# IRIS-AUDIO/SELD

Measured on AMD Instinct MI355X. Metric: train-step clips/sec (7ch×3000×64) seldnet.json at 1/2/4/8 MI355X, higher is better.
Workload: dtype f32; 1 GPU; model_config/seldnet.json train step (fwd+BCE/MSE+bwd+Adam), 32 clips/GPU of [T=3000,F=64,C=7], n_classes=12; global_batch=32, parallelism=dp1, dp_backend=none

## Files before the change

### seld_amd/csrc/api.hip

```cpp
#include "ctx.h"

#include <algorithm>
#include <math.h>
#include <stdio.h>
#include <string.h>

static std::string g_create_err;

int fail(seld_ctx* c, int code, const std::string& msg) {
    if (c) c->err = msg; else g_create_err = msg;
    return code;
}

static void add_var(std::vector<Var>& v, int64_t& off, const std::string& name, std::initializer_list<int64_t> shape) {
    Var x;
    x.name = name;
    x.off = off;
    x.rank = (int)shape.size();
    int64_t n = 1;
    int i = 0;
    for (int k = 0; k < 4; ++k) x.shape[k] = 1;
    for (auto s : shape) { x.shape[i++] = s; n *= s; }
    off += n;
    v.push_back(x);
// ... 357 lines not shown
        return fail(nullptr, SELD_ERR_HIP, "side stream / event creation failed");
    }
    for (int i = 0; i < a->n_gru; ++i)
        if (hipEventCreateWithFlags(&c->ev_bucket[i], hipEventDisableTiming) != hipSuccess) {
            seld_destroy(c);
            return fail(nullptr, SELD_ERR_HIP, "event creation failed");
        }
    ALLOC(c->sync_buf, (resn ? 16 * 128 : 128) + 1);
    for (int hd = 0; hd < 2; ++hd)
        for (auto& D : c->heads[hd].layers) {
            ALLOC(D.y, rows * (size_t)D.out); ALLOC(D.dy, rows * (size_t)D.out);
            if (D.ks > 1) ALLOC(D.xe, rows * (size_t)D.in);
            if (D.rate > 0.f) ALLOC(D.yd, rows * (size_t)D.out);
        }
    {
        size_t tmp = 0;
        for (int hd = 0; hd < 2; ++hd) for (auto& D : c->heads[hd].layers) if (D.ks > 1) tmp = std::max(tmp, rows * (size_t)D.in);
        if (tmp) ALLOC(c->head_tmp, tmp);
        if (a->output_coupling) ALLOC(c->doa_v1, rows * (size_t)(3 * a->n_classes));
    }
    {
        size_t ne = 0;
        for (int i = 0; i < a->n_gru; ++i) ne += 4 * gemm_sb_split_elems(c->gru[i].in_feat, 384);
        for (int hd = 0; hd < 2; ++hd) ne += 2 * gemm_sb_split_elems(c->heads[hd].layers[0].in, c->heads[hd].layers[0].out);
        ALLOC(c->gsplit, ne);
        unsigned short* q = c->gsplit;
        for (int i = 0; i < a->n_gru; ++i)
            for (int d = 0; d < 2; ++d) {
                c->ksp_fwd[i][d] = q; q += gemm_sb_split_elems(c->gru[i].in_feat, 384);
                c->ksp_bwd[i][d] = q; q += gemm_sb_split_elems(c->gru[i].in_feat, 384);
            }
        for (int hd = 0; hd < 2; ++hd) {
            const DenseL& D = c->heads[hd].layers[0];
            c->h0sp_fwd[hd] = q; q += gemm_sb_split_elems(D.in, D.out);
            c->h0sp_bwd[hd] = q; q += gemm_sb_split_elems(D.in, D.out);
        }
    }
    {
        const int nt = c->heads[0].layers.back().out + c->heads[1].layers.back().out, k = c->heads[0].layers[0].in;
        ALLOC(c->weff, (size_t)(k + 1) * nt);
        ALLOC(c->dy_all, rows * (size_t)nt);
        ALLOC(c->headF, (size_t)k * nt + nt);
    }
    ALLOC(c->loss_scratch, (size_t)loss_scratch_floats((int)rows));
    ALLOC(c->den_dev, 4); ALLOC(c->loss_out, rows + 4);
#undef ALLOC
    { int rc_ = v2_tables_create(c); if (rc_) { g_create_err = c->err; seld_destroy(c); return rc_; } }
    if (hipDeviceSynchronize() != hipSuccess) { seld_destroy(c); return fail(nullptr, SELD_ERR_HIP, "device sync after allocation failed"); }
    *out = c;
    return SELD_OK;
}

void seld_destroy(seld_ctx* c) {
    if (!c) return;
    hipSetDevice(c->device);
    hipDeviceSynchronize();
    for (auto& t : c->timers) for (auto e : t.ev) hipEventDestroy(e);
    for (auto e : c->ev_pool) hipEventDestroy(e);
    if (c->ev_fork) hipEventDestroy(c->ev_fork);
    if (c->ev_join) hipEventDestroy(c->ev_join);
    if (c->ev_prep) hipEventDestroy(c->ev_prep);
    if (c->ev_gram) hipEventDestroy(c->ev_gram);
    if (c->ev_rn_ready) hipEventDestroy(c->ev_rn_ready);
    for (auto e_ : c->ev_rn_free) if (e_) hipEventDestroy(e_);
    for (auto e : c->ev_bucket) if (e) hipEventDestroy(e);
    seld_dp_destroy(c);
    if (c->side) hipStreamDestroy(c->side);
    for (void* p : c->allocs) hipFree(p);
    delete c;
}

int seld_set_stream(seld_ctx* c, void* s) { if (!c) return SELD_ERR_INVALID; c->stream = (hipStream_t)s; return SELD_OK; }
int seld_set_batch(seld_ctx* c, int B) {
    if (!c) return SELD_ERR_INVALID;
    if (B < 1 || B > c->Bmax) return fail(c, SELD_ERR_INVALID, "batch exceeds the size given to seld_create");
    c->B = B;
    return SELD_OK;
}
int seld_set_option(seld_ctx* c, const char* key, int value) {
    if (!c || !key) return SELD_ERR_INVALID;
    if (!strcmp(key, "conv64_split_bf16")) { c->conv64_split_bf16 = value != 0; return SELD_OK; }
    if (!strcmp(key, "gemm_split_bf16")) { c->gemm_split_bf16 = value != 0; return SELD_OK; }
    if (!strcmp(key, "heads_fused")) { c->heads_fused = value != 0; return SELD_OK; }
    if (!strcmp(key, "dropout_seed")) { c->dropout_seed = 0x5e1d5e1d00000000ull ^ (uint64_t)(unsigned)value; return SELD_OK; }
    if (!strcmp(key, "dropout_step")) { c->dropout_step = (unsigned)value; return SELD_OK; }
    if (!strcmp(key, "conv1_split_bf16")) { c->conv1_split_bf16 = value != 0; return SELD_OK; }
    if (!strcmp(key, "gram_bg_blocks") && value >= 16 && value <= 512) { c->gram_bg_blocks = value; return SELD_OK; }
    if (!strcmp(key, "conv1_pool_fused")) { c->conv1_pool_fused = value != 0; return SELD_OK; }
    if (!strcmp(key, "conv1_gram")) { c->conv1_gram = value != 0; return SELD_OK; }
    if (!strcmp(key, "gru_wgrad_batch")) { c->gru_wgrad_batch = value != 0; return SELD_OK; }
    if (!strcmp(key, "gru_din_first")) { c->gru_din_first = value != 0; return SELD_OK; }
    if (!strcmp(key, "conv2_pre_fused")) { c->conv2_pre_fused = value != 0; return SELD_OK; }
    if (!strcmp(key, "conv3_pre_fused")) { c->conv3_pre_fused = value != 0; return SELD_OK; }
    if (!strcmp(key, "gram_parts") && (value == 1 || value == 2)) { c->gram_parts = value; return SELD_OK; }
    if (!strcmp(key, "xc_fused_fwd")) { c->xc_fused_fwd = value != 0; return SELD_OK; }
    if (!strcmp(key, "rn_split_bf16")) { c->rn_split_bf16 = value != 0; return SELD_OK; }
    if (!strcmp(key, "rn_wgrad_side")) { c->rn_wgrad_side = value != 0; return SELD_OK; }
    if (!strcmp(key, "rn_implicit3x3")) { c->rn_implicit3x3 = value != 0; return SELD_OK; }
    if (!strcmp(key, "rn_epi_stats")) { c->rn_epi_stats = value != 0; return SELD_OK; }
    if (!strcmp(key, "rn_epi_add")) { c->rn_epi_add = value != 0; return SELD_OK; }
    if (!strcmp(key, "xc_wgrad_side")) { c->xc_wgrad_side = value != 0; return SELD_OK; }
    if (!strcmp(key, "xc_fused_pw_bwd")) { c->xc_fused_pw_bwd = value != 0; return SELD_OK; }
    if (!strcmp(key, "bwd_four_products")) { c->bwd_four_products = value != 0; return SELD_OK; }
    if (!strcmp(key, "tn_tile_blocks") && value >= 64 && value <= 4096) { c->tn_tile_blocks = value; return SELD_OK; }
    if (!strcmp(key, "gru_var")) {
        if (value < 0 || value > 255) return fail(c, SELD_ERR_INVALID, "gru_var: 0..255");
        c->gru_var = value; return SELD_OK;
    }
    if (!strcmp(key, "tn_lds_floor") && value >= 0 && value <= 100) { c->tn_lds_floor = value; return SELD_OK; }
    if (!strcmp(key, "conv64_dbuf")) { c->conv64_dbuf = value != 0; return SELD_OK; }
    if (!strcmp(key, "conv_wgrad_side")) { c->conv_wgrad_side = value != 0; return SELD_OK; }
    if (!strcmp(key, "dgrad_r8")) { c->dgrad_r8 = value != 0; return SELD_OK; }
    if (!strcmp(key, "prep_side")) { c->prep_side = value != 0; return SELD_OK; }
    if (!strcmp(key, "xc_nowait")) { c->xc_nowait = value != 0; return SELD_OK; }
    if (!strcmp(key, "xc_fused_bn_sums")) { c->xc_fused_bn_sums = value != 0; return SELD_OK; }
    if (!strcmp(key, "xc_fused_dw_bwd")) { c->xc_fused_dw_bwd = value != 0; return SELD_OK; }
    if (!strcmp(key, "xc_w16")) { c->xc_w16 = value != 0; return SELD_OK; }
    if (!strcmp(key, "xc_xcd_map")) { c->xc_xcd_map = value != 0; return SELD_OK; }
    if (!strcmp(key, "bf16_single")) { c->bf16_single = value != 0; return SELD_OK; }
    return fail(c, SELD_ERR_INVALID, std::string("unknown option: ") + key);
}
int seld_sync(seld_ctx* c) {
    if (!c) return SELD_ERR_INVALID;
    HIPCHK(c, hipStreamSynchronize(c->stream));
    return SELD_OK;
}

int64_t seld_param_count(const seld_ctx* c) { return c ? c->nparam : -1; }
int64_t seld_state_count(const seld_ctx* c) { return c ? c->nstate : -1; }
int seld_variable_count(const seld_ctx* c, int trainable) { return c ? (int)(trainable ? c->tr.size() : c->nt.size()) : -1; }
int seld_variable_info(const seld_ctx* c, int trainable, int index, char* name, int name_cap, int64_t* offset,
                       int32_t* rank, int64_t shape[4]) {
    if (!c) return SELD_ERR_INVALID;
    const std::vector<Var>& v = trainable ? c->tr : c->nt;
    if (index < 0 || index >= (int)v.size()) return SELD_ERR_INVALID;
    if (name && name_cap > 0) { strncpy(name, v[index].name.c_str(), name_cap - 1); name[name_cap - 1] = 0; }
    if (offset) *offset = v[index].off;
    if (rank) *rank = v[index].rank;
    if (shape) for (int k = 0; k < 4; ++k) shape[k] = v[index].shape[k];
    return SELD_OK;
}

static int copy_h2d(seld_ctx* c, float* dst, const float* src, int64_t n, int64_t expect) {
    if (!c || !src || n != expect) return fail(c, SELD_ERR_INVALID, "size mismatch in host->device copy");
    HIPCHK(c, hipStreamSynchronize(c->stream));
    HIPCHK(c, hipMemcpy(dst, src, (size_t)n * 4, hipMemcpyHostToDevice));
    return SELD_OK;
}
static int copy_d2h(seld_ctx* c, float* dst, const float* src, int64_t n, int64_t expect) {
    if (!c || !dst || n != expect) return fail(c, SELD_ERR_INVALID, "size mismatch in device->host copy");
    HIPCHK(c, hipStreamSynchronize(c->stream));
    HIPCHK(c, hipMemcpy(dst, src, (size_t)n * 4, hipMemcpyDeviceToHost));
    return SELD_OK;
}
int seld_set_weights_host(seld_ctx* c, const float* w, int64_t n) { return c ? copy_h2d(c, c->params, w, n, c->nparam) : SELD_ERR_INVALID; }
int seld_get_weights_host(seld_ctx* c, float* w, int64_t n) { return c ? copy_d2h(c, w, c->params, n, c->nparam) : SELD_ERR_INVALID; }
int seld_set_state_host(seld_ctx* c, const float* s, int64_t n) { return c ? copy_h2d(c, c->state, s, n, c->nstate) : SELD_ERR_INVALID; }
int seld_get_state_host(seld_ctx* c, float* s, int64_t n) { return c ? copy_d2h(c, s, c->state, n, c->nstate) : SELD_ERR_INVALID; }
int seld_get_grads_host(seld_ctx* c, float* g, int64_t n) { return c ? copy_d2h(c, g, c->grads, n, c->nparam) : SELD_ERR_INVALID; }
int seld_get_adam_host(seld_ctx* c, float* m, float* v, int64_t n) {
    if (!c) return SELD_ERR_INVALID;
    int rc = copy_d2h(c, m, c->adam_m, n, c->nparam);
    if (rc) return rc;
    return copy_d2h(c, v, c->adam_v, n, c->nparam);
}
int seld_set_adam_host(seld_ctx* c, const float* m, const float* v, int64_t n, int64_t step) {
    if (!c || step < 0) return SELD_ERR_INVALID;
    int rc = copy_h2d(c, c->adam_m, m, n, c->nparam);
    if (rc) return rc;
    rc = copy_h2d(c, c->adam_v, v, n, c->nparam);
    if (rc) return rc;
    c->adam_step = step;
    return SELD_OK;
}
void* seld_param_ptr(seld_ctx* c) { return c ? c->params : nullptr; }
void* seld_grad_ptr(seld_ctx* c) { return c ? c->grads : nullptr; }

int seld_forward(seld_ctx* c, const float* x, float* sed, float* doa, int training) {
    if (!c || !x) return SELD_ERR_INVALID;
    HIPCHK(c, hipSetDevice(c->device));
    return forward_impl(c, x, sed, doa, training, false);
}

static int run_losses(seld_ctx* c, const float* y_sed, const float* y_doa, const seld_loss_cfg* cfg, float* sloss,
                      float* dloss, bool want_grads, bool defer_finalize = false) {
    hipStream_t st = c->stream;
    const int rows = c->B * c->S, nc = c->arch.n_classes;
    if (cfg->doa_loss < SELD_DOA_MSE || cfg->doa_loss > SELD_DOA_MSLE) return fail(c, SELD_ERR_INVALID, "bad doa_loss");
    if (cfg->doa_loss == SELD_DOA_MMSE) {
        if (cfg->mmse_den > 0.f) {
            if (hipMemcpyAsync(c->den_dev, &cfg->mmse_den, 4, hipMemcpyHostToDevice, st) != hipSuccess)
                return fail(c, SELD_ERR_HIP, "den copy failed");
            hipStreamSynchronize(st);
        } else {
            launch_mmse_den(st, y_doa, c->den_dev, c->loss_scratch, rows, nc);
            if (want_grads && c->dp_comm && c->dp_world > 1 && dp_allreduce(c, c->den_dev, 1, SELD_DTYPE_F32, st)) return fail(c, SELD_ERR_HIP, "RCCL all-reduce of the MMSE denominator failed");
        }
    }
    float* sl = sloss ? sloss : c->loss_out;
    float* dl = dloss ? dloss : c->loss_out + 4;
    const bool lin = heads_lin(c);
    const int n0 = c->heads[0].layers.back().out, nt = n0 + c->heads[1].layers.back().out;
    launch_losses(st, c->heads[0].layers.back().y, c->arch.output_coupling ? c->doa_v1 : c->heads[1].layers.back().y, y_sed, y_doa, cfg->doa_loss, cfg->w_sed,
                  cfg->w_doa, cfg->sed_grad_scale, c->den_dev, sl, dl,
                  want_grads ? (lin ? c->dy_all : c->heads[0].layers.back().dy) : nullptr,
                  want_grads ? (lin ? c->dy_all + n0 : c->heads[1].layers.back().dy) : nullptr, c->loss_scratch, c->B, c->S, nc,
                  lin ? nt : 0, lin ? nt : 0, defer_finalize ? 1 : 0);
    if (want_grads && c->arch.output_coupling)
        launch_v1_couple_bwd(st, c->heads[0].layers.back().y, c->heads[1].layers.back().y, lin ? c->dy_all : c->heads[0].layers.back().dy,
                             lin ? nt : n0, lin ? c->dy_all + n0 : c->heads[1].layers.back().dy, lin ? nt : nt - n0, rows, nc);
    if (defer_finalize) { c->fin_sl = sl; c->fin_dl = dl; c->fin_doa_loss = cfg->doa_loss; }
    return check_launch(c, "losses");
}

int seld_mmse_den(seld_ctx* c, const float* y_doa, float* den) {
    if (!c || !y_doa || !den) return SELD_ERR_INVALID;
    HIPCHK(c, hipSetDevice(c->device));
    launch_mmse_den(c->stream, y_doa, den, c->loss_scratch, c->B * c->S, c->arch.n_classes);
    return check_launch(c, "mmse_den");
}

int seld_test_step(seld_ctx* c, const float* x, const float* y_sed, const float* y_doa, const seld_loss_cfg* cfg,
                   float* sed, float* doa, float* sloss, float* dloss) {
    if (!c || !x || !y_sed || !y_doa || !cfg) return SELD_ERR_INVALID;
    HIPCHK(c, hipSetDevice(c->device));
    int rc = forward_impl(c, x, sed, doa, 0, false);
    if (rc) return rc;
    return run_losses(c, y_sed, y_doa, cfg, sloss, dloss, false);
}

int seld_train_fwd_bwd(seld_ctx* c, const float* x, const float* y_sed, const float* y_doa, const seld_loss_cfg* cfg,
                       float* sed, float* doa, float* sloss, float* dloss) {
    if (!c || !x || !y_sed || !y_doa || !cfg) return SELD_ERR_INVALID;
    HIPCHK(c, hipSetDevice(c->device));
    int rc = forward_impl(c, x, sed, doa, 1, true);
    if (rc) return rc;
    rc = run_losses(c, y_sed, y_doa, cfg, sloss, dloss, true, true);
    if (rc) return rc;
    return backward_impl(c, x);
}

int seld_adam_step(seld_ctx* c, float lr, float beta1, float beta2, float eps, int agc) {
    if (!c) return SELD_ERR_INVALID;
    HIPCHK(c, hipSetDevice(c->device));
    if (agc)
        for (auto& v : c->tr) launch_agc(c->stream, c->params, c->grads, v.off, v.rank, v.shape, nullptr);
    c->adam_step += 1;
    const double t = (double)c->adam_step;
    const float lr_t = (float)((double)lr * sqrt(1.0 - pow((double)beta2, t)) / (1.0 - pow((double)beta1, t)));
    PROF2(c, "adam");
    launch_adam(c->stream, c->params, c->grads, c->adam_m, c->adam_v, c->nparam, lr_t, beta1, beta2, eps);
    return check_launch(c, "adam");
}

int seld_train_step(seld_ctx* c, const float* x, const float* y_sed, const float* y_doa, const seld_loss_cfg* cfg,
                    float lr, int agc, float* sed, float* doa, float* sloss, float* dloss) {
    int rc = seld_train_fwd_bwd(c, x, y_sed, y_doa, cfg, sed, doa, sloss, dloss);
    if (rc) return rc;
    return seld_adam_step(c, lr, 0.9f, 0.999f, 1e-7f, agc);
}

int seld_debug_pool_routing(seld_ctx* c, int block, unsigned char* pos, unsigned char* gate) {
    if (c && pos && gate && c->arch.first_kind == SELD_FIRST_XCEPTION && block == (int)c->conv.size()) {
        HIPCHK(c, hipSetDevice(c->device));
        if (launch_pool_routing(c->stream, c->xc_x.back(), c->xc_feat, nullptr, c->xc_ident + 128, c->xc_ident + 192, pos, gate, c->B, c->S, 16, 1, 8))
            return fail(c, SELD_ERR_UNSUPPORTED, "pool_routing");
        HIPCHK(c, hipStreamSynchronize(c->stream));
        return check_launch(c, "pool_routing");
    }
    if (!c || !pos || !gate || block < 0 || block >= (int)c->conv.size()) return SELD_ERR_INVALID;
    HIPCHK(c, hipSetDevice(c->device));
    const ConvL& L = c->conv[block];
    const bool recorded = block == 0 && L.amax && (c->gram_active || (L.pf == 4 && (L.pt == 5 || L.pt == 4 || L.pt == 2 || L.pt == 1)));
    if (launch_pool_routing(c->stream, L.z, L.p, recorded ? L.amax : nullptr, L.scale, L.shift, pos, gate, c->B, L.H, L.W, L.pt, L.pf))
        return fail(c, SELD_ERR_UNSUPPORTED, "pool_routing");
    HIPCHK(c, hipStreamSynchronize(c->stream));
    return check_launch(c, "pool_routing");
}

static int set_override(seld_ctx* c, int kind, int block, int which, int64_t n, const int64_t* idx_host, const unsigned char* val_host, int64_t limit) {
    HIPCHK(c, hipSetDevice(c->device));
    HIPCHK(c, hipStreamSynchronize(c->stream));
    for (size_t i = 0; i < c->overrides.size();)
        if (c->overrides[i].kind == kind && c->overrides[i].block == block && c->overrides[i].which == which) c->overrides.erase(c->overrides.begin() + i);
        else ++i;
    if (n <= 0) return SELD_OK;
    if (!idx_host || !val_host) return SELD_ERR_INVALID;
    for (int64_t k = 0; k < n; ++k)
        if (idx_host[k] < 0 || idx_host[k] >= limit) return fail(c, SELD_ERR_INVALID, "injected decision index out of range");
    seld_ctx::Override o{kind, block, which, n, nullptr, nullptr};
    if (dalloc(c, &o.idx, (size_t)n) || dalloc(c, &o.val, (size_t)n)) return SELD_ERR_NOMEM;
    HIPCHK(c, hipMemcpy(o.idx, idx_host, (size_t)n * sizeof(int64_t), hipMemcpyHostToDevice));
    HIPCHK(c, hipMemcpy(o.val, val_host, (size_t)n, hipMemcpyHostToDevice));
    c->overrides.push_back(o);
    return SELD_OK;
}

int seld_debug_set_routing(seld_ctx* c, int block, int64_t n, const int64_t* idx_host, const unsigned char* val_host) {
    if (c && c->arch.first_kind == SELD_FIRST_XCEPTION && block == (int)c->conv.size()) {
        for (int64_t k = 0; k < n && val_host; ++k)
            if (val_host[k] > 8) return fail(c, SELD_ERR_INVALID, "injected routing value exceeds 1 + the window size");
        return set_override(c, 3, block, 0, n, idx_host, val_host, (int64_t)c->Bmax * c->S * 2 * 64);
    }
    if (!c || block < 0 || block >= (int)c->conv.size()) return SELD_ERR_INVALID;
    const ConvL& L = c->conv[block];
    const int64_t limit = (int64_t)c->Bmax * (L.H / L.pt) * (L.W / L.pf) * 64;
    for (int64_t k = 0; k < n && val_host; ++k)
        if (val_host[k] > L.pt * L.pf) return fail(c, SELD_ERR_INVALID, "injected routing value exceeds 1 + the window size");
    return set_override(c, 0, block, 0, n, idx_host, val_host, limit);
}

int seld_debug_set_relu_gates(seld_ctx* c, int block, int which, int64_t n, const int64_t* idx_host, const unsigned char* val_host) {
    if (!c || which < 0 || which > 2) return SELD_ERR_INVALID;
    if (c->arch.first_kind == SELD_FIRST_XCEPTION) {
        if (block < 0 || block >= (int)c->xc.size() || which != 0) return SELD_ERR_INVALID;
        return set_override(c, 2, block, 0, n, idx_host, val_host, (int64_t)c->Bmax * c->S * 16 * 64);
    }
    if (c->arch.first_kind != SELD_FIRST_RESNET50 || block < 0 || block >= (int)c->rn.size()) return SELD_ERR_INVALID;
    const RnBlock& R = c->rn[block];
    const int64_t limit = (int64_t)c->Bmax * c->S * R.Wout * (which == 2 ? 4 * R.w : R.w);
// ... 68 lines not shown
```

### seld_amd/csrc/backward.hip

```cpp
#include "ctx.h"

#include <algorithm>
#include <stdio.h>

static void wgrad_dense(seld_ctx* c, hipStream_t st, float* slab, const float* A, int lda, const float* Bm, int ldb, int M,
                        int K1, int N, int64_t w_off, int64_t b_off, int S, int shift) {
    int ns = 0;
    const int64_t cap = tn_slab_capacity() / ((int64_t)K1 * N + N);
    if (c->gemm_split_bf16 && gemm_tn_sb_usable(A, lda, Bm, ldb, K1, N)) launch_gemm_tn_sb(st, A, lda, Bm, ldb, slab, &ns, M, N, S, shift, 1);
    else launch_gemm_tn(st, A, lda, Bm, ldb, slab, &ns, M, K1, N, S, shift, 1, (int)std::min<int64_t>(cap, gemm_tn_max_splits()));
    launch_reduce_slabs2(st, slab, ns, (int64_t)K1 * N + N, c->grads + w_off, (int64_t)K1 * N, c->grads + b_off, N);
}

static void rn_bn_bwd(seld_ctx* c, hipStream_t st, RnConv& cv, const float* dy, const unsigned char* gate4, float* dz, int64_t M) {
    int nbx = 0;
    const int gate_z = gate4 ? 2 : 1;
    const float* mask = reinterpret_cast<const float*>(gate4);
    launch_rn_bn_bwd_reduce(st, cv.z, dy, mask, cv.coef, c->rn_part, &nbx, M, cv.Cout, gate_z);
    if (c->sync_fn) {
        const int nd = (cv.Cout + 63) / 64 * 128;
        launch_rn_bn_bwd_finalize(st, c->rn_part, nbx, (double)M, c->grads + cv.g_off, c->grads + cv.be_off, cv.coef, cv.Cout, c->sync_buf, 1);
        if (c->sync_fn(c->sync_user, c->sync_buf, nd + 1, SELD_DTYPE_F64, st)) { c->sync_failed = true; return; }
        launch_rn_bn_bwd_finalize(st, c->rn_part, nbx, 0.0, c->grads + cv.g_off, c->grads + cv.be_off, cv.coef, cv.Cout, c->sync_buf, 2);
    } else
        launch_rn_bn_bwd_finalize(st, c->rn_part, nbx, (double)M, c->grads + cv.g_off, c->grads + cv.be_off, cv.coef, cv.Cout);
    launch_rn_bn_bwd_dz(st, cv.z, dy, mask, cv.coef, dz, M, cv.Cout, gate_z);
}

static void heads_lin_side(seld_ctx* c, int rows) {
    const DenseL& S0 = c->heads[0].layers[0];
    const GruL& Glast = c->gru.back();
    const int nt = c->heads[0].layers[1].out + c->heads[1].layers[1].out, K = S0.in;
    int ns = 0;
    launch_gemm_tn(c->side, Glast.out, K, c->dy_all, nt, c->tn_slab_side, &ns, rows, K, nt, 0, 0, 1);
    launch_reduce_slabs2(c->side, c->tn_slab_side, ns, (int64_t)K * nt + nt, c->headF, (int64_t)K * nt, c->headF + (size_t)K * nt, nt);
    const float *w1[2], *b1[2], *w2[2];
    float *dw1[2], *db1[2], *dw2[2], *db2[2];
    int n[2];
    for (int hd = 0; hd < 2; ++hd) {
        const DenseL &L0 = c->heads[hd].layers[0], &L1 = c->heads[hd].layers[1];
        w1[hd] = c->params + L0.w_off; b1[hd] = c->params + L0.b_off; w2[hd] = c->params + L1.w_off;
        dw1[hd] = c->grads + L0.w_off; db1[hd] = c->grads + L0.b_off; dw2[hd] = c->grads + L1.w_off; db2[hd] = c->grads + L1.b_off;
        n[hd] = L1.out;
    }
    launch_heads_grad(c->side, w1, b1, w2, dw1, db1, dw2, db2, n, K, S0.out, c->headF, c->headF + (size_t)K * nt);
}

static int apply_overrides(seld_ctx* c) {
    hipStream_t st = c->stream;
    for (const auto& o : c->overrides) {
        if (o.kind == 0) {
            ConvL& L = c->conv[o.block];
            const bool recorded = o.block == 0 && L.amax && (c->gram_active || (L.pf == 4 && (L.pt == 5 || L.pt == 4 || L.pt == 2 || L.pt == 1)));
            if (!recorded && !L.z) return fail(c, SELD_ERR_UNSUPPORTED, "seld_debug_set_routing: this block keeps neither recorded positions nor its pre-BN tensor");
            launch_pool_routing_patch(st, L.z, L.p, recorded ? L.amax : nullptr, L.scale, L.shift, o.idx, o.val, o.n, L.H, L.W, L.pt, L.pf);
        } else if (o.kind == 2) {
            const int b = o.block / 3, u = o.block % 3;
            const bool fold = c->xc_fused_fwd && u > 0;
            if (fold) launch_relu_gate_patch_z(st, c->xc[o.block - 1].z, nullptr, c->xc[o.block - 1].scale, c->xc[o.block - 1].scale + 64, 64, o.idx, o.val, o.n);
            else launch_relu_gate_patch(st, u == 0 ? c->xc_x[b] : c->xc[o.block - 1].a, nullptr, o.idx, o.val, o.n);
        } else if (o.kind == 3) {
            launch_pool_routing_patch(st, c->xc_x.back(), c->xc_feat, nullptr, c->xc_ident + 128, c->xc_ident + 192, o.idx, o.val, o.n, c->S, 16, 1, 8);
        } else {
            RnBlock& R = c->rn[o.block];
            if (o.which == 2) launch_relu_gate_patch(st, R.out, R.gate, o.idx, o.val, o.n);
            else {
                RnConv& K = R.c[o.which];
                launch_relu_gate_patch_z(st, K.z, o.which == 0 ? R.y0 : R.y1, K.coef + 2 * K.Cout, K.coef + 3 * K.Cout, K.Cout, o.idx, o.val, o.n);
            }
        }
    }
    return SELD_OK;
}

static int backward_heads(seld_ctx* c) {
    hipStream_t st = c->stream;
    const int rows = c->B * c->S;
    GruL& Glast = c->gru.back();
    PROF2(c, "heads_bwd");
    float* dfeat = c->feat_grad;
    DenseL &S0 = c->heads[0].layers[0], &D0 = c->heads[1].layers[0];
    if (heads_lin(c)) {
        const int nt = c->heads[0].layers[1].out + c->heads[1].layers[1].out, K = S0.in;
        launch_gemm(st, c->dy_all, nt, c->weff, nt, nullptr, dfeat, K, rows, K, nt, 1, 0, 0);
    } else if (heads_general(c)) {
        for (int hd = 0; hd < 2; ++hd) {
            Head& Hd = c->heads[hd];
            for (int j = (int)Hd.layers.size() - 1; j >= 0; --j) {
                DenseL& D = Hd.layers[j];
                float* din = j == 0 ? dfeat : Hd.layers[j - 1].dy;
                const int accumulate = (j == 0 && hd == 1) ? 1 : 0;
                if (D.ks > 1) {
                    launch_gemm(st, D.dy, D.out, c->params + D.w_off, D.out, nullptr, c->head_tmp, D.in, rows, D.in, D.out, 1, 0, 0);
                    launch_time_fold(st, c->head_tmp, din, c->B, c->S, D.in_base, D.ks, accumulate);
                } else {
                    launch_gemm(st, D.dy, D.out, c->params + D.w_off, D.out, nullptr, din, D.in, rows, D.in, D.out, 1, 0, accumulate);
                }
                if (j > 0) {
                    const DenseL& P = Hd.layers[j - 1];
                    const int64_t n = (int64_t)rows * P.out;
                    if (P.rate > 0.f && c->last_training) launch_dropout(st, din, din, n, P.rate, c->dropout_seed, P.drop_id, c->dropout_cur);
                    if (Hd.hidden_act) launch_act_bwd(st, P.y, din, n, Hd.hidden_act);
                }
            }
        }
        fork_side(c);
        for (int hd = 0; hd < 2; ++hd) {
            Head& Hd = c->heads[hd];
            for (int j = (int)Hd.layers.size() - 1; j >= 0; --j) {
                DenseL& D = Hd.layers[j];
                const float* ain = D.ks > 1 ? D.xe
                                 : (j == 0 ? Glast.out : (Hd.layers[j - 1].rate > 0.f && c->last_training ? Hd.layers[j - 1].yd : Hd.layers[j - 1].y));
                wgrad_dense(c, c->side, c->tn_slab_side, ain, D.in, D.dy, D.out, rows, D.in, D.out, D.w_off, D.b_off, 0, 0);
            }
        }
    } else {
    const bool merged0 = S0.in == D0.in && S0.out == D0.out && (S0.out & 31) == 0;
    for (int hd = 0; hd < 2; ++hd) {
        Head& Hd = c->heads[hd];
        for (int j = (int)Hd.layers.size() - 1; j >= (merged0 ? 1 : 0); --j) {
            DenseL& D = Hd.layers[j];
            float* din = j == 0 ? dfeat : Hd.layers[j - 1].dy;
            const int accumulate = (j == 0 && hd == 1) ? 1 : 0;
            launch_gemm(st, D.dy, D.out, c->params + D.w_off, D.out, nullptr, din, D.in, rows, D.in, D.out, 1, 0, accumulate);
            if (j > 0 && Hd.hidden_act) launch_act_bwd(st, Hd.layers[j - 1].y, din, (int64_t)rows * D.in, Hd.hidden_act);
        }
    }
    if (merged0 && heads_sb(c) && gemm_sb_usable(S0.dy, S0.out, S0.in, S0.out) && gemm_sb_usable(D0.dy, S0.out, S0.in, S0.out)) {
        BwdFourScope four_;
        launch_gemm_sb(st, S0.dy, D0.dy, S0.out, c->h0sp_bwd[0], c->h0sp_bwd[1], nullptr, nullptr, dfeat, nullptr, S0.in, rows, S0.in,
                       S0.out, 0, 2);
    } else if (merged0)
        launch_gemm_dual_k(st, S0.dy, D0.dy, S0.out, c->params + S0.w_off, c->params + D0.w_off, S0.out, nullptr, dfeat, S0.in, rows,
                           S0.in, S0.out, 1, 0, 0);
    fork_side(c);
    for (int hd = 0; hd < 2; ++hd) {
        Head& Hd = c->heads[hd];
        for (int j = (int)Hd.layers.size() - 1; j >= 0; --j) {
            DenseL& D = Hd.layers[j];
            const float* ain = j == 0 ? Glast.out : Hd.layers[j - 1].y;
            wgrad_dense(c, c->side, c->tn_slab_side, ain, D.in, D.dy, D.out, rows, D.in, D.out, D.w_off, D.b_off, 0, 0);
        }
    }
    }
    return SELD_OK;
}

static int backward_gru(seld_ctx* c, const float* dfeat, const float** din) {
    hipStream_t st = c->stream;
    const int B = c->B, S = c->S, rows = B * S;
    const float* dout = dfeat;
    for (int i = (int)c->gru.size() - 1; i >= 0; --i) {
        GruL& G = c->gru[i];
        const bool conv_drop = c->last_training && c->arch.conv_dropout > 0.f, gru_drop = c->last_training && c->arch.gru_dropout > 0.f;
        const float* lin = i == 0 ? (c->arch.first_kind == SELD_FIRST_XCEPTION ? c->xc_feat : (c->arch.first_kind == SELD_FIRST_RESNET50 ? c->rn.back().out : (conv_drop ? c->conv.back().pd : c->conv.back().p))) : c->gru[i - 1].out;
        {
            PROF(c, "gru_bwd");
            if (gru_drop) {
// ... 369 lines not shown
```

### seld_amd/csrc/common.h

```cpp
#pragma once
#include <hip/hip_runtime.h>
#include <stdint.h>
#include "../../include/seld_hip.h"

inline int ok() { return hipGetLastError() == hipSuccess ? SELD_OK : SELD_ERR_HIP; }

typedef float f32x16 __attribute__((ext_vector_type(16)));

#define MFMA_F32_32x32x2(a, b, c) __builtin_amdgcn_mfma_f32_32x32x2f32((a), (b), (c), 0, 0, 0)

__device__ __forceinline__ int mfma_row(int r, int hi) { return (r & 3) + 8 * (r >> 2) + 4 * hi; }

__device__ __forceinline__ f32x16 zero16() {
    f32x16 z;
#pragma unroll
    for (int i = 0; i < 16; ++i) z[i] = 0.f;
    return z;
}
__device__ __forceinline__ float dpp_quad_xor1(float v) {
    return __int_as_float(__builtin_amdgcn_update_dpp(0, __float_as_int(v), 0xB1 , 0xF, 0xF, true));
}
__device__ __forceinline__ float dpp_quad_xor2(float v) {
    return __int_as_float(__builtin_amdgcn_update_dpp(0, __float_as_int(v), 0x4E , 0xF, 0xF, true));
}
// ... 152 lines not shown
int launch_rn_product_fwd(hipStream_t st, const float* A, int lda, const float* w, const unsigned short* wsp, float* z, int M, int K, int N,
                          float* stat_part = nullptr, int* nbx = nullptr, size_t part_cap = 0);
int launch_rn_product_dgrad(hipStream_t st, const float* dz, const float* w, const unsigned short* wsp_t, float* dA, int ldd, int M, int K, int N,
                            int accumulate, const float* addg = nullptr, const unsigned char* gate4 = nullptr);
int launch_rn_product_wgrad(hipStream_t st, const float* A, int lda, const float* dz, float* slab, int64_t slab_cap, float* dw, int M, int K, int N,
                            int split_bf16);
int launch_rn_w32_embed(hipStream_t st, const float* w, float* w2);
int launch_rn_w32_extract(hipStream_t st, const float* dw2, float* dw);
int rn_conv3_sb_ok(int C, int N);
int launch_rn_conv3_fwd(hipStream_t st, const float* img, const unsigned short* wsp, float* z, int B, int H, int W, int C, int N,
                        float* stat_part = nullptr, int* nbx = nullptr, size_t part_cap = 0);
int launch_rn_conv3_dgrad(hipStream_t st, const float* dz, const unsigned short* wsp_flip, float* dimg, int B, int H, int W, int C, int N);
int launch_rn_conv3_wgrad(hipStream_t st, const float* img, const float* dz, float* slab, int64_t slab_cap, float* dw, int B, int H, int W, int C, int N);
int launch_xc_unit_fwd(hipStream_t st, const float* x, const float* kdw, const float* wpw, float* dwo, float* z, float* partial, int* npartial,
                       int B, int H, int W, const float* aff = nullptr);
int xc_partial_capacity();
int launch_dw3x3_fwd(hipStream_t st, const float* x, const float* k, float* y, int B, int H, int W, const float* aff = nullptr);
int launch_dw3x3_bwd_data(hipStream_t st, const float* dy, const float* k, const float* xin, const float* add, float* dx, int B, int H, int W,
                          const float* aff = nullptr);
int launch_dw3x3_bwd_w(hipStream_t st, const float* x, const float* dy, float* slab, int* nslab, int B, int H, int W, const float* aff = nullptr);
int xc_dw_fused_slabs(int B, int H);
int launch_dw3x3_bwd_fused(hipStream_t st, const float* dy, const float* k, const float* xin, const float* add, float* dx, float* slab, int* nslab,
                           int B, int H, int W, const float* aff = nullptr, const float* bn_mean = nullptr, const float* bn_invstd = nullptr,
                           float* bn_partial = nullptr);
int launch_xc_fold_partials(hipStream_t st, const float* partial, int n, float* out, int* nout);
int launch_xc_bn_stats(hipStream_t st, const float* z, float* partial, int* npartial, int64_t npix);
int launch_xc_bn_bwd_reduce(hipStream_t st, const float* z, const float* dy, const float* mean, const float* invstd, float* partial,
                            int* npartial, int64_t npix);
int launch_xc_bn_apply(hipStream_t st, const float* z, const float* scale, const float* shift, const float* res, float* out, int64_t npix);
int xc_pw_bwd_slabs();
int launch_xc_pw_bwd(hipStream_t st, const float* z, const float* gy, const float* dwo, const float* wpw, const float* mean, const float* invstd,
                     const float* scale, const float* c1c2, float* f1, float* slab, int* nslab, int64_t npix);
int launch_xc_bn_bwd_dz(hipStream_t st, const float* z, const float* dy, const float* mean, const float* invstd, const float* scale,
                        const float* c1c2, float* dz, int64_t npix);
int launch_xc_ident(hipStream_t st, float* ident);
int launch_bn_partials_to_sums(hipStream_t st, const float* partial, int npartial, double* sums, double local_count);
int launch_bn_finalize_sums(hipStream_t st, const double* sums, double count, const float* gamma, const float* beta,
                            float* mov_mean, float* mov_var, float* mean, float* invstd, float* scale, float* shift);
int launch_bn_bwd_local(hipStream_t st, const double* sums, float* dgamma, float* dbeta);
int launch_bn_bwd_c1c2(hipStream_t st, const double* sums, double count, float* c1c2);
int launch_pool_routing_patch(hipStream_t st, float* z, float* p, unsigned char* amax, const float* scale, const float* shift,
                              const int64_t* idx, const unsigned char* val, int64_t n, int H, int W, int pt, int pf);
int launch_relu_gate_patch_z(hipStream_t st, float* z, float* y, const float* scale, const float* shift, int C, const int64_t* idx,
                             const unsigned char* val, int64_t n);
int launch_affine_copy(hipStream_t st, const float* x, const float* aff, float* dst, int64_t n, int C);
int launch_relu_gate_patch(hipStream_t st, float* y, unsigned char* gate_bits, const int64_t* idx, const unsigned char* val, int64_t n);
int launch_pool_routing(hipStream_t st, const float* z, const float* p, const unsigned char* amax, const float* scale,
                        const float* shift, unsigned char* pos, unsigned char* gate, int B, int H, int W, int pt, int pf);
int launch_bn_pool_bwd_dz(hipStream_t st, const float* z, const float* dp, const float* mean, const float* invstd,
                          const float* scale, const float* shift, const float* c1c2, float* dz,
                          int B, int H, int W, int C, int pt, int pf);
int bn_partial_capacity();

struct GemmEpi { float* stat_part = nullptr; const float* addg = nullptr; const unsigned char* gate4 = nullptr; };
extern thread_local GemmEpi g_gemm_epi;
struct GemmEpiScope {
    GemmEpiScope(float* stat_part, const float* addg = nullptr, const unsigned char* gate4 = nullptr) { g_gemm_epi.stat_part = stat_part; g_gemm_epi.addg = addg; g_gemm_epi.gate4 = gate4; }
    ~GemmEpiScope() { g_gemm_epi = GemmEpi(); }
};
int gemm_epi_row_blocks(int M, int split_bf16);
int launch_gemm(hipStream_t st, const float* A, int lda, const float* Bm, int ldb, const float* bias, float* C,
                int ldc, int M, int N, int K, int transb, int act, int accumulate);
int launch_gemm_dual_n(hipStream_t st, const float* A, int lda, const float* B0, const float* B1, int ldb, const float* bias0,
                       const float* bias1, float* C0, float* C1, int ldc, int M, int N, int K, int transb, int act);
int launch_gemm_mirror(hipStream_t st, const float* A, int lda, const float* Bm, int ldb, const float* bias, float* C, float* mirror,
                       int ldc, int M, int N, int K, int transb, int act);
int launch_gemm_heads(hipStream_t st, const float* A, int lda, const float* Bm, const float* bias, float* C0, float* C1, float* M0,
                      float* M1, int M, int n0, int n1, int K, int act0, int act1);
int launch_heads_weff(hipStream_t st, const float* const* w1, const float* const* b1, const float* const* w2, const float* const* b2,
                      const int* n, int K, int Hd, float* weff);
int launch_heads_grad(hipStream_t st, const float* const* w1, const float* const* b1, const float* const* w2, float* const* dw1,
                      float* const* db1, float* const* dw2, float* const* db2, const int* n, int K, int Hd, const float* F,
                      const float* cs);
int launch_gemm_dual_k(hipStream_t st, const float* A0, const float* A1, int lda, const float* B0, const float* B1, int ldb,
                       const float* bias, float* C, int ldc, int M, int N, int K, int transb, int act, int accumulate);
extern int g_gsb_dbg;
size_t gemm_sb_split_elems(int K, int N);
int gemm_sb_usable(const void* A, int lda, int N, int K);
int launch_gemm_split_b(hipStream_t st, int njobs, const float* const* src, unsigned short* const* dst, const int* ldb,
                        const int* transb, const int* K, const int* N);
int launch_gemm_sb(hipStream_t st, const float* A0, const float* A1, int lda, const unsigned short* Bs0, const unsigned short* Bs1,
                   const float* bias0, const float* bias1, float* C0, float* C1, int ldc, int M, int N, int K, int act, int mode,
                   int accum = 0,
                   int conv_C = 0, int conv_H = 0, int conv_W = 0);
int launch_gemm_tn(hipStream_t st, const float* A, int lda, const float* Bm, int ldb, float* slab, int* nslab,
                   int M, int K1, int N, int S, int shift, int want_bias, int max_splits = 0, int chunk_rows = 32);
int gemm_tn_sb_usable(const void* A, int lda, const void* Bm, int ldb, int K1, int N);
#define TN_MAX_JOBS 4
struct TnJobs {
    const float* A[TN_MAX_JOBS];
    const float* B[TN_MAX_JOBS];
    int lda[TN_MAX_JOBS], shift[TN_MAX_JOBS];
    float* out_w[TN_MAX_JOBS];
    float* out_b[TN_MAX_JOBS];
};
int launch_gemm_tn_sb_batch(hipStream_t st, const TnJobs& jobs, int njobs, int ldb, float* slab, int* nslab, int M, int N, int S, int want_bias);
int launch_reduce_slabs2_batch(hipStream_t st, const float* slab, int nslab, int64_t stride, const TnJobs& jobs, int njobs, int64_t n_w, int64_t n_b);
int launch_gemm_tn_sb(hipStream_t st, const float* A, int lda, const float* Bm, int ldb, float* slab, int* nslab, int M, int N, int S,
                      int shift, int want_bias);
int launch_gemm_tn_sb_tiles(hipStream_t st, const float* A, int lda, const float* Bm, int ldb, float* slab, int64_t slab_cap, int* nslab,
                            int M, int K1, int N, int conv_C = 0, int conv_H = 0, int conv_W = 0);
int launch_reduce_slabs2(hipStream_t st, const float* slab, int nslab, int64_t stride, float* out_w, int64_t n_w,
                         float* out_b, int64_t n_b);
int gemm_tn_max_splits();
inline int64_t tn_slab_capacity() { return (int64_t)gemm_tn_max_splits() * (384 * 384 + 384); }
int launch_colsum(hipStream_t st, const float* X, int ld, float* slab, int* nslab, int M, int N);

int launch_gru_fwd(hipStream_t st, const float* gx_f, const float* gx_b, const float* U_f, const float* U_b,
                   const float* brec_f, const float* brec_b, float* h_f, float* h_b, float* sv_f, float* sv_b,
                   int B, int S, const float* rm_f = nullptr, const float* rm_b = nullptr, float* hm_f = nullptr, float* hm_b = nullptr);
int launch_gru_fwd_df(hipStream_t st, const float* gx_f, const float* gx_b, const float* U_f, const float* U_b,
                      const float* brec_f, const float* brec_b, float* h_f, float* h_b, float* sv_f, float* sv_b, int B, int S);
int gru_df_trace_read(int which, unsigned long long* out);
int launch_gru_bwd(hipStream_t st, const float* dout, const float* h_f, const float* h_b, const float* sv_f,
                   const float* sv_b, const float* U_f, const float* U_b, float* dgx_f, float* dgx_b,
                   float* dgh_f, float* dgh_b, int B, int S, const float* rm_f = nullptr, const float* rm_b = nullptr, const float* hm_f = nullptr,
                   const float* hm_b = nullptr);
int gru_timing_read(int which, unsigned long long* out, int blocks);
int launch_gru_fwd_uni(hipStream_t st, const float* gx, const float* U, const float* brec, float* h, float* sv, int B, int S);
int launch_gru_bwd_dh(hipStream_t st, const float* dh_f, const float* dh_b, const float* h_f, const float* h_b, const float* sv_f, const float* sv_b,
                      const float* U_f, const float* U_b, float* dgx_f, float* dgx_b, float* dgh_f, float* dgh_b, int B, int S);
int launch_lstm_fwd(hipStream_t st, const float* gx_f, const float* gx_b, const float* U_f, const float* U_b, float* h_f, float* h_b,
                    float* c_f, float* c_b, float* sv_f, float* sv_b, int B, int S);
int launch_lstm_bwd(hipStream_t st, const float* dh_f, const float* dh_b, const float* c_f, const float* c_b, const float* sv_f,
                    const float* sv_b, const float* U_f, const float* U_b, float* dgx_f, float* dgx_b, int B, int S);
int launch_mul(hipStream_t st, const float* a, const float* b, float* out, int64_t n);

struct seld_loss_cfg;
int launch_act_bwd(hipStream_t st, const float* y, float* dy, int64_t n, int act);
int launch_time_expand(hipStream_t st, const float* x, float* xe, int B, int S, int C, int ks);
int launch_time_fold(hipStream_t st, const float* dxe, float* dx, int B, int S, int C, int ks, int accumulate);
int launch_dropout(hipStream_t st, const float* in, float* out, int64_t n, float rate, uint64_t seed, unsigned layer, unsigned step);
int launch_mask_rows(hipStream_t st, const float* in, const float* mask, float* out, int64_t rows, int S, int F, int accumulate);
int launch_fill(hipStream_t st, float* out, int64_t n, float v);
int launch_v1_couple_fwd(hipStream_t st, const float* sed, const float* doa1, float* out, float* out2, int rows, int nc);
int launch_v1_couple_bwd(hipStream_t st, const float* sed, const float* doa1, float* dsed_pre, int ld_sed, float* ddoa_pre, int ld_doa, int rows, int nc);
int launch_mmse_den(hipStream_t st, const float* y_doa, float* den, float* scratch, int rows, int nc);
int launch_losses(hipStream_t st, const float* sed, const float* doa, const float* y_sed, const float* y_doa,
                  int doa_loss, float w_sed, float w_doa, float sed_grad_scale, const float* den_dev,
                  float* sloss, float* dloss, float* dsed_pre, float* ddoa_pre, float* scratch, int B, int S, int nc, int ld_sed = 0,
                  int ld_doa = 0, int defer_finalize = 0);
int launch_losses_finalize(hipStream_t st, int doa_loss, const float* den_dev, float* sloss, float* dloss, float* scratch, int B, int S,
                           int nc);
int loss_scratch_floats(int rows);
int launch_adam(hipStream_t st, float* theta, const float* g, float* m, float* v, int64_t n, float lr_t,
                float beta1, float beta2, float eps);
int launch_agc(hipStream_t st, const float* theta, float* g, int64_t off, int rank, const int64_t* shape,
               float* scratch);
```

### seld_amd/csrc/ctx.h

```cpp
#pragma once
#include "common.h"
#include "../../include/seld_hip.h"

#include <string>
#include <vector>

struct Var { std::string name; int64_t off; int rank; int64_t shape[4]; };

struct Timer { std::string name; std::vector<hipEvent_t> ev; int64_t launches = 0; double ms = 0.0; };

struct ConvL {
    int H, W, Cin, pt, pf;
    int64_t w_off, b_off, g_off, be_off;
    int64_t mm_off, mv_off;
    float *z = nullptr, *p = nullptr, *dp = nullptr;
    float* pd = nullptr;
    unsigned char* amax = nullptr;
    float* zext = nullptr;
    float *mean, *invstd, *scale, *shift, *c1c2;
};

struct GruL {
    int in_feat;
    int64_t k_off[2], u_off[2], b_off[2];
// ... 13 lines not shown
    unsigned short *wsp = nullptr, *wsp_t = nullptr;
    unsigned short *wsp9 = nullptr, *wsp9_flip = nullptr;
    float *w2 = nullptr, *dw2 = nullptr;
};
struct RnBlock {
    int Cin, w, stride_f, Win, Wout;
    bool proj;
    RnConv c[3], sc;
    float *y0 = nullptr, *y1 = nullptr, *out = nullptr;
    unsigned char* gate = nullptr;
};

struct XcUnit {
    int64_t dw_off, pw_off, g_off, be_off;
    int64_t mm_off, mv_off;
    float *dwo = nullptr, *z = nullptr, *a = nullptr;
    float *mean, *invstd, *scale, *shift, *c1c2;
};

struct Head {
    std::vector<DenseL> layers;
    int act;
    int hidden_act = 0;
};

struct seld_ctx {
    seld_arch arch;
    int B, Bmax, T, S, device;
    hipStream_t stream = nullptr;
    std::vector<Var> tr, nt;
    int64_t nparam = 0, nstate = 0;
    float *params = nullptr, *grads = nullptr, *adam_m = nullptr, *adam_v = nullptr, *state = nullptr;
    int64_t adam_step = 0;
    std::vector<ConvL> conv;
    std::vector<GruL> gru;
    struct Override { int kind, block, which; int64_t n; int64_t* idx; unsigned char* val; };
    std::vector<Override> overrides;
    Head heads[2];
    std::vector<XcUnit> xc;
    std::vector<float*> xc_x;
    float *xc_small = nullptr, *xc_ident = nullptr, *xc_feat = nullptr, *xc_part = nullptr, *xc_slab = nullptr;
    float* xc_unit_slab = nullptr;
    size_t xc_unit_slab_per = 0, xc_unit_slab_pw = 0, xc_unit_slab_dw = 0;
    int xc_nowait = 1;
    float* xc_slab_tmp = nullptr;
    float* xc_part_dw = nullptr;
    size_t xc_slab_per = 0;
    float *xc_g[4] = {}, *xc_dz2 = nullptr;
    int xc_fused_pw_bwd = 1;
    int xc_wgrad_side = 1;
    std::vector<RnBlock> rn;
    float *rn_part = nullptr, *rn_part_side = nullptr, *rn_gx[2] = {}, *rn_bz[2] = {}, *rn_ba = nullptr, *rn_bb[3] = {}, *rn_bcol = nullptr;
    size_t rn_part_floats = 0;
    hipEvent_t ev_rn_ready = nullptr, ev_rn_free[5] = {};
    float* rn_w9_slab = nullptr;
    int rn_wgrad_side = 1;
    size_t rn_col_elems = 0;
    int rn_implicit3x3 = 1;
    int rn_feat = 0;
    float *feat_grad = nullptr;
    float *dzbuf = nullptr, *small = nullptr, *stat_partial = nullptr, *bn_partial = nullptr;
    float *wgrad_slab = nullptr, *tn_slab = nullptr, *cs_slab = nullptr, *wflip = nullptr;
    float *wgrad_slab_side = nullptr, *dzbuf_alt = nullptr;
    int conv_wgrad_side = 1;
    int dgrad_r8 = 1;
    float *dgx[SELD_MAX_LAYERS][2] = {}, *dgh[SELD_MAX_LAYERS][2] = {};
    float* tn_slab_side = nullptr;
    unsigned short* wsplit = nullptr;
    unsigned short *wsp_fwd[SELD_MAX_LAYERS] = {}, *wsp_bwd[SELD_MAX_LAYERS] = {};
    int conv1_gram = 1;
    bool xc_fused_fwd = true;
    int gram_parts = 2;
    bool conv3_pre_fused = true;
    bool conv2_pre_fused = true;
    bool gru_din_first = false;
    bool gru_wgrad_batch = true;
    bool gram_active = false;
    float *gram_slab = nullptr, *gram = nullptr, *mmat = nullptr;
    hipEvent_t ev_gram = nullptr;
    int conv1_split_bf16 = 1;
    int conv1_pool_fused = 1;
    int heads_fused = 1;
    float *weff = nullptr, *dy_all = nullptr, *headF = nullptr;
    int rn_split_bf16 = 1;
    int gemm_split_bf16 = 1;
    unsigned short* gsplit = nullptr;
    unsigned short *ksp_fwd[SELD_MAX_LAYERS][2] = {}, *ksp_bwd[SELD_MAX_LAYERS][2] = {}, *h0sp_fwd[2] = {}, *h0sp_bwd[2] = {};
    int conv64_split_bf16 = 1;
    hipStream_t side = nullptr;
    hipEvent_t ev_fork = nullptr, ev_join = nullptr, ev_prep = nullptr;
    int prep_side = 0;
    hipEvent_t ev_bucket[SELD_MAX_LAYERS] = {};
    seld_allreduce_fn sync_fn = nullptr;
    void* sync_user = nullptr;
    int sync_world = 1;
    double* sync_buf = nullptr;
    bool sync_failed = false;
    int bf16_single = 0;
    int bwd_four_products = 1, gru_var = 11, conv64_dbuf = 1, tn_tile_blocks = 384, tn_lds_floor = 0, gram_bg_blocks = 192;
    int xc_fused_bn_sums = 1;
    int xc_fused_dw_bwd = 1;
    int xc_w16 = 1;
    int xc_xcd_map = 1;
    int rn_epi_stats = 1;
    int rn_epi_add = 1;
    void* dp_comm = nullptr;
    int dp_rank = 0, dp_world = 1;
    hipStream_t dp_stream = nullptr;
    hipEvent_t ev_dp_main = nullptr, ev_dp_done = nullptr;
    float *dsed_pre = nullptr, *ddoa_pre = nullptr, *sed_int = nullptr, *doa_int = nullptr;
    float *doa_v1 = nullptr;
    float *head_tmp = nullptr;
    float* ones = nullptr;
    uint64_t dropout_seed = 0x5e1d5e1d5e1d5e1dull; unsigned dropout_step = 0, dropout_cur = 0; int last_training = 0;
    float *loss_scratch = nullptr, *den_dev = nullptr, *loss_out = nullptr;
    float *fin_sl = nullptr, *fin_dl = nullptr;
    int fin_doa_loss = 0;
    struct V2Tab { void *tiles = nullptr, *segs = nullptr; int32_t* reg = nullptr; float* scale = nullptr; int ntiles = 0, nsegs = 0; } v2;
    float *swa_w = nullptr, *swa_s = nullptr;
    int swa_cnt = 0;
    std::vector<void*> allocs;
    std::string err;
    int prof = 0;
    std::vector<Timer> timers;
    std::vector<hipEvent_t> ev_pool;
};

int fail(seld_ctx* c, int code, const std::string& msg);
int check_launch(seld_ctx* c, const char* what);

#define HIPCHK(c, expr)                                                                         \
    do {                                                                                        \
        hipError_t e_ = (expr);                                                                 \
        if (e_ != hipSuccess)                                                                   \
            return fail(c, SELD_ERR_HIP, std::string(#expr) + ": " + hipGetErrorString(e_));    \
    } while (0)

template <typename T>
int dalloc(seld_ctx* c, T** p, size_t n) {
    void* q = nullptr;
    hipError_t e = hipMalloc(&q, n * sizeof(T) + 256);
    if (e != hipSuccess) return fail(c, SELD_ERR_NOMEM, std::string("hipMalloc: ") + hipGetErrorString(e));
    c->allocs.push_back(q);
    *p = reinterpret_cast<T*>(q);
    return 0;
}

struct ProfScope {
    seld_ctx* c; int idx;
    ProfScope(seld_ctx* c_, const char* name, int level = 1) : c(c_), idx(-1) {
        if (c->prof < level) return;
        for (size_t i = 0; i < c->timers.size(); ++i) if (c->timers[i].name == name) idx = (int)i;
        if (idx < 0) { Timer t; t.name = name; c->timers.push_back(t); idx = (int)c->timers.size() - 1; }
        hipEvent_t e = take(c); hipEventRecord(e, c->stream); c->timers[idx].ev.push_back(e);
    }
    ~ProfScope() {
        if (idx < 0) return;
        hipEvent_t e = take(c); hipEventRecord(e, c->stream); c->timers[idx].ev.push_back(e);
        c->timers[idx].launches++;
    }
    static hipEvent_t take(seld_ctx* c) {
        if (c->ev_pool.empty()) { hipEvent_t e; hipEventCreate(&e); return e; }
        hipEvent_t e = c->ev_pool.back(); c->ev_pool.pop_back(); return e;
    }
};
#define PROF_CAT2(a, b) a##b
#define PROF_CAT(a, b) PROF_CAT2(a, b)
#define PROF(c, name) ProfScope PROF_CAT(prof_scope_, __LINE__)(c, name, 1)
#define PROF2(c, name) ProfScope PROF_CAT(prof_scope_, __LINE__)(c, name, 2)
#define PROF3(c, name) ProfScope PROF_CAT(prof_scope_, __LINE__)(c, name, 3)

void fork_side(seld_ctx* c);
void apply_kernel_choices(const seld_ctx* c);
bool gru_sb(const seld_ctx* c, const GruL& G);
bool heads_general(const seld_ctx* c);
bool heads_sb(const seld_ctx* c);
bool heads_lin(const seld_ctx* c);
bool rn_c1_implicit(const seld_ctx* c, const RnBlock& R);
int rn_c1_width(const RnBlock& R);
bool rn_c1_direct(const RnBlock& R);

int forward_impl(seld_ctx* c, const float* x, float* sed, float* doa, int training, bool save);
int backward_impl(seld_ctx* c, const float* x);

int v2_tables_create(seld_ctx* c);

int dp_allreduce(seld_ctx* c, void* buf, int64_t count, int dtype, hipStream_t st);
```

### seld_amd/csrc/forward.hip

```cpp
#include "ctx.h"

#include <stdio.h>

static int prepare_heads_weff(seld_ctx* c, hipStream_t st) {
    const float *w1[2], *b1[2], *w2[2], *b2[2];
    int n[2];
    for (int hd = 0; hd < 2; ++hd) {
        const DenseL &L0 = c->heads[hd].layers[0], &L1 = c->heads[hd].layers[1];
        w1[hd] = c->params + L0.w_off; b1[hd] = c->params + L0.b_off; w2[hd] = c->params + L1.w_off; b2[hd] = c->params + L1.b_off;
        n[hd] = L1.out;
    }
    return launch_heads_weff(st, w1, b1, w2, b2, n, c->heads[0].layers[0].in, c->heads[0].layers[0].out, c->weff);
}

static int prepare_gemm_splits(seld_ctx* c, hipStream_t st, bool with_grad_orientation) {
    const float* src[16]; unsigned short* dst[16]; int ldb[16], tb[16], K[16], N[16];
    int n = 0;
    auto flush = [&]() { int rc = n ? launch_gemm_split_b(st, n, src, dst, ldb, tb, K, N) : 0; n = 0; return rc; };
    auto add = [&](const float* w, unsigned short* d, int ld, int transb, int k, int nn) {
        src[n] = w; dst[n] = d; ldb[n] = ld; tb[n] = transb; K[n] = k; N[n] = nn;
        return ++n == 16 ? flush() : 0;
    };
    for (size_t i = 0; i < c->gru.size(); ++i) {
        const GruL& G = c->gru[i];
// ... 3 lines not shown
            if (with_grad_orientation && add(c->params + G.k_off[d], c->ksp_bwd[i][d], 384, 1, 384, G.in_feat)) return -1;
        }
    }
    if (heads_sb(c) && !heads_lin(c))
        for (int hd = 0; hd < 2; ++hd) {
            const DenseL& D = c->heads[hd].layers[0];
            if (add(c->params + D.w_off, c->h0sp_fwd[hd], D.out, 0, D.in, D.out)) return -1;
            if (with_grad_orientation && add(c->params + D.w_off, c->h0sp_bwd[hd], D.out, 1, D.out, D.in)) return -1;
        }
    return flush();
}

static void rn_bn(seld_ctx* c, hipStream_t st, RnConv& cv, int64_t M, int training, int nbx_have = 0, float* part = nullptr) {
    int nbx = nbx_have;
    if (!part) part = c->rn_part;
    if (training && !nbx_have) launch_rn_bn_stats(st, cv.z, part, &nbx, M, cv.Cout);
    float *g = c->params + cv.g_off, *be = c->params + cv.be_off, *mm = c->state + cv.mm_off, *mv = c->state + cv.mv_off;
    if (training && c->sync_fn) {
        const int nd = (cv.Cout + 63) / 64 * 128;
        launch_rn_bn_finalize(st, part, nbx, (double)M, g, be, mm, mv, cv.coef, cv.Cout, 1, c->sync_buf, 1);
        if (c->sync_fn(c->sync_user, c->sync_buf, nd + 1, SELD_DTYPE_F64, st)) { c->sync_failed = true; return; }
        launch_rn_bn_finalize(st, part, nbx, 0.0, g, be, mm, mv, cv.coef, cv.Cout, 1, c->sync_buf, 2);
        return;
    }
    launch_rn_bn_finalize(st, part, nbx, (double)M, g, be, mm, mv, cv.coef, cv.Cout, training);
}

static int heads_couple(seld_ctx* c, float* doa, int rows) {
    if (c->arch.output_coupling)
        launch_v1_couple_fwd(c->stream, c->heads[0].layers.back().y, c->heads[1].layers.back().y, c->doa_v1, doa, rows, c->arch.n_classes);
    return check_launch(c, "forward");
}

static void rn_weight_prep(seld_ctx* c, hipStream_t st, bool save) {
    const float* src[16]; unsigned short* dst[16]; int ldb[16], tb[16], Ks[16], Ns[16];
    int n = 0;
    auto add = [&](const float* w, unsigned short* d, int ld, int transb, int k, int nn) {
        src[n] = w; dst[n] = d; ldb[n] = ld; tb[n] = transb; Ks[n] = k; Ns[n] = nn;
        if (++n == 16) { launch_gemm_split_b(st, n, src, dst, ldb, tb, Ks, Ns); n = 0; }
    };
    for (auto& R : c->rn)
        for (RnConv* cv : {&R.c[0], &R.c[1], &R.c[2], &R.sc}) {
            const int K = cv->k * cv->k * cv->Cin, N = cv->Cout;
            if (cv->wsp) add(c->params + cv->w_off, cv->wsp, N, 0, K, N);
            if (cv->wsp_t && save) {
                if (cv == &R.c[1] && rn_c1_implicit(c, R)) add(c->params + cv->w_off, cv->wsp_t, N, 2, 9 * N, cv->Cin);
                else add(c->params + cv->w_off, cv->wsp_t, N, 1, N, K);
            }
        }
    if (n) launch_gemm_split_b(st, n, src, dst, ldb, tb, Ks, Ns);
    const float* w9[8]; unsigned short* d9[8]; int f9[8];
    n = 0;
    for (auto& R : c->rn) {
        if (!rn_c1_direct(R)) continue;
        const float* wsrc = c->params + R.c[1].w_off;
        if (R.c[1].w2) { launch_rn_w32_embed(st, wsrc, R.c[1].w2); wsrc = R.c[1].w2; }
        w9[n] = wsrc; d9[n] = R.c[1].wsp9; f9[n++] = 0;
        if (save) { w9[n] = wsrc; d9[n] = R.c[1].wsp9_flip; f9[n++] = 1; }
        if (n >= 7) { launch_split_weights_batch(st, n, w9, d9, f9); n = 0; }
    }
    if (n) launch_split_weights_batch(st, n, w9, d9, f9);
}

template <typename Layer>
static int bn_coeffs(seld_ctx* c, hipStream_t st, int training, const float* part, int np, double count, Layer& L) {
    const float *g = c->params + L.g_off, *be = c->params + L.be_off;
    float *mm = c->state + L.mm_off, *mv = c->state + L.mv_off;
    if (training && c->sync_fn) {
        launch_bn_partials_to_sums(st, part, np, c->sync_buf, count);
        if (c->sync_fn(c->sync_user, c->sync_buf, 129, SELD_DTYPE_F64, st)) return fail(c, SELD_ERR_HIP, "sync_bn all-reduce callback failed");
        launch_bn_finalize_sums(st, c->sync_buf, 0.0 , g, be, mm, mv, L.mean, L.invstd, L.scale, L.shift);
    } else if (training)
        launch_bn_finalize(st, part, np, count, g, be, mm, mv, L.mean, L.invstd, L.scale, L.shift, 64, 1);
    else
        launch_bn_eval_coeffs(st, g, be, mm, mv, L.scale, L.shift, 64);
    return SELD_OK;
}

struct FwdPass {
    const float* x;
    int training;
    bool save;
    bool conv_drop, gru_drop;
};

static int forward_weight_prep(seld_ctx* c, bool save, bool* prep_on_side, bool* rn_prep_on_side) {
    hipStream_t st = c->stream;
    *prep_on_side = false;
    *rn_prep_on_side = !c->rn.empty() && c->rn_split_bf16 && c->prep_side && c->ev_prep;
    if (*rn_prep_on_side) { fork_side(c); rn_weight_prep(c, c->side, save); hipEventRecord(c->ev_prep, c->side); }
    GemmSplitJobs a; SplitWeightJobs b; HeadsLin h;
    a.one = b.one = g_mfma_one;
    int na = 0, nb = 0;
    bool fits = true;
    auto adda = [&](const float* w, unsigned short* d, int ld, int transb, int k, int nn) {
        if (na == GSB_MAX_JOBS) { fits = false; return; }
        a.src[na] = w; a.dst[na] = d; a.ldb[na] = ld; a.transb[na] = transb; a.K[na] = k; a.N[na] = nn; ++na;
    };
    for (size_t i = 0; i < c->gru.size(); ++i) {
        const GruL& G = c->gru[i];
        if (!gru_sb(c, G)) continue;
        for (int d = 0; d < 2; ++d) {
            adda(c->params + G.k_off[d], c->ksp_fwd[i][d], 384, 0, G.in_feat, 384);
            if (save) adda(c->params + G.k_off[d], c->ksp_bwd[i][d], 384, 1, 384, G.in_feat);
        }
    }
    if (heads_sb(c) && !heads_lin(c))
        for (int hd = 0; hd < 2; ++hd) {
            const DenseL& D = c->heads[hd].layers[0];
            adda(c->params + D.w_off, c->h0sp_fwd[hd], D.out, 0, D.in, D.out);
            if (save) adda(c->params + D.w_off, c->h0sp_bwd[hd], D.out, 1, D.out, D.in);
        }
    a.njobs = na;
    static_assert(2 * (SELD_MAX_LAYERS - 1) <= 8, "the conv64 weight planes of a step fit one SplitWeightJobs");
    if (c->conv64_split_bf16)
        for (size_t i = 1; i < c->conv.size(); ++i) {
            b.w[nb] = c->params + c->conv[i].w_off; b.dst[nb] = c->wsp_fwd[i]; b.flip[nb++] = 0;
            if (save) { b.w[nb] = c->params + c->conv[i].w_off; b.dst[nb] = c->wsp_bwd[i]; b.flip[nb++] = 1; }
        }
    const bool lin = heads_lin(c);
    if (lin)
        for (int hd = 0; hd < 2; ++hd) {
            const DenseL &L0 = c->heads[hd].layers[0], &L1 = c->heads[hd].layers[1];
            h.w1[hd] = c->params + L0.w_off; h.b1[hd] = c->params + L0.b_off; h.w2[hd] = c->params + L1.w_off;
            h.b2[hd] = c->params + L1.b_off; h.n[hd] = L1.out;
            h.K = L0.in; h.Hd = L0.out;
        }
    if (fits && (!lin || h.K + 1 <= 4 * 144)) {
        *prep_on_side = c->prep_side && c->ev_prep && c->xc.empty() && c->rn.empty() && c->conv.size() >= 2;
        if (*prep_on_side) fork_side(c);
        if (launch_weight_prep(*prep_on_side ? c->side : st, a, na, b, nb, h, lin ? c->weff : nullptr)) return fail(c, SELD_ERR_UNSUPPORTED, "weight_prep");
        if (*prep_on_side) hipEventRecord(c->ev_prep, c->side);
    } else {
        if (prepare_gemm_splits(c, st, save)) return fail(c, SELD_ERR_UNSUPPORTED, "gemm_split_b");
        if (lin && prepare_heads_weff(c, st)) return fail(c, SELD_ERR_UNSUPPORTED, "heads_weff");
        if (nb && launch_split_weights_batch(st, nb, b.w, b.dst, b.flip)) return fail(c, SELD_ERR_UNSUPPORTED, "split_weights");
    }
    return SELD_OK;
}

static int forward_conv_blocks(seld_ctx* c, const FwdPass& p, bool prep_on_side, const float** feat) {
    hipStream_t st = c->stream;
    const int B = c->B;
    const float* in = p.x;
    bool pre_pending = false;
    for (size_t i = 0; i < c->conv.size(); ++i) {
        ConvL& L = c->conv[i];
        bool ext_now = false;
        int npart = 0;
        float* stat = p.training ? c->stat_partial : nullptr;
        char tn[32];
        snprintf(tn, sizeof tn, "conv%d_fwd", (int)i + 1);
        const bool fused_pool = i == 0 && c->conv1_pool_fused && L.pt == 5 && L.pf == 4 && L.W == 64;
        const bool gram = fused_pool && p.save && c->conv1_gram;
        if (i == 0) c->gram_active = gram;
        const bool pre_next = fused_pool && (gram || !p.save) && c->conv2_pre_fused && !p.conv_drop && c->arch.first_kind == SELD_FIRST_SIMPLE_CONV &&
                              i + 1 < c->conv.size() && c->conv64_split_bf16 && !g_mfma_one && conv64_fwd_sb_takes_pre(c->conv[i + 1].W);
        if (fused_pool) {
            PROF(c, tn);
            if (launch_conv_first_fwd_pool(st, in, c->params + L.w_off, c->params + L.b_off, c->params + L.g_off,
                                           (p.save && !gram) ? L.z : nullptr, (gram || pre_next) ? L.zext : L.p, p.save ? L.amax : nullptr, stat,
                                           &npart, B, L.H, L.Cin, c->conv1_split_bf16))
                return fail(c, SELD_ERR_UNSUPPORTED, "conv_first_fwd_pool");
        } else if (i == 0) {
            PROF(c, tn);
            if (launch_conv_first_fwd(st, in, c->params + L.w_off, c->params + L.b_off, L.z, stat, &npart, B, L.H, L.Cin))
                return fail(c, SELD_ERR_UNSUPPORTED, "conv_first_fwd");
// ... 84 lines not shown
        if (rn_prep_on_side) hipStreamWaitEvent(st, c->ev_prep, 0);
        else rn_weight_prep(c, st, p.save);
    }
    const float* X = *feat;
    int rc_ = 0;
    for (auto& R : c->rn) {
        if (c->sync_failed) break;
        const int64_t M = (int64_t)B * S * R.Wout;
        const int w = R.w;
        const bool sc_side = R.proj && c->rn_wgrad_side && !c->sync_fn;
        if (sc_side) {
            hipEventRecord(c->ev_rn_ready, st); hipStreamWaitEvent(c->side, c->ev_rn_ready, 0);
            int nb_ = 0;
            if (launch_rn_product_fwd(c->side, X, R.Cin * R.stride_f, c->params + R.sc.w_off, sb ? R.sc.wsp : nullptr, R.sc.z, (int)M, R.Cin, 4 * w,
                                      epi_stats ? c->rn_part_side : nullptr, &nb_, c->rn_part_floats))
                return fail(c, SELD_ERR_INVALID, "resnet50_block: projection shortcut product refused");
            rn_bn(c, c->side, R.sc, M, p.training, nb_, c->rn_part_side);
            hipEventRecord(c->ev_rn_free[0], c->side);
        }
        int nb0 = 0;
        { PROF3(c, "rn_products_fwd"); rc_ = launch_rn_product_fwd(st, X, R.Cin * R.stride_f, c->params + R.c[0].w_off, sb ? R.c[0].wsp : nullptr, R.c[0].z, (int)M, R.Cin, w,
                                                                   epi_stats ? c->rn_part : nullptr, &nb0, c->rn_part_floats); }
        if (rc_) return fail(c, SELD_ERR_INVALID, "resnet50_block: reduce convolution's product refused");
        { PROF3(c, "rn_bn_fwd"); rn_bn(c, st, R.c[0], M, p.training, nb0); }
        { PROF3(c, "rn_bn_fwd"); launch_rn_bn_apply(st, R.c[0].z, R.c[0].coef, nullptr, R.y0, M, w, 1); }
        if (sb && rn_c1_direct(R)) {
            int npart = 0;
            if (R.c[1].w2) {
                { PROF3(c, "rn_products_fwd"); launch_conv64_fwd_sb(st, R.y0, R.c[1].wsp9, nullptr, R.c[1].z, nullptr, nullptr, B, S, rn_c1_width(R)); }
                { PROF3(c, "rn_bn_fwd"); rn_bn(c, st, R.c[1], M, p.training); }
            } else {
                if (p.training && (size_t)conv_sb_partial_capacity() * 128 > c->rn_part_floats)
                    return fail(c, SELD_ERR_INVALID, "resnet50_block: more BatchNorm partials than rn_part holds");
                { PROF3(c, "rn_products_fwd"); launch_conv64_fwd_sb(st, R.y0, R.c[1].wsp9, nullptr, R.c[1].z, p.training ? c->rn_part : nullptr, &npart, B, S, R.Wout); }
                { PROF3(c, "rn_bn_fwd"); rn_bn(c, st, R.c[1], M, p.training, npart); }
            }
        } else if (sb && rn_c1_implicit(c, R)) {
            int nb1 = 0;
            { PROF3(c, "rn_products_fwd"); rc_ = launch_rn_conv3_fwd(st, R.y0, R.c[1].wsp, R.c[1].z, B, S, R.Wout, w, w, epi_stats ? c->rn_part : nullptr, &nb1,
                                                                     c->rn_part_floats); }
            if (rc_) return fail(c, SELD_ERR_INVALID, "resnet50_block: 3x3 convolution's product refused");
            { PROF3(c, "rn_bn_fwd"); rn_bn(c, st, R.c[1], M, p.training, nb1); }
        } else {
            if (!R.c[1].col && dalloc(c, &R.c[1].col, (size_t)M * 9 * w)) return fail(c, SELD_ERR_NOMEM, "im2col tensor");
            launch_im2col3x3(st, R.y0, R.c[1].col, B, S, R.Wout, w);
            int nb1 = 0;
            { PROF3(c, "rn_products_fwd"); rc_ = launch_rn_product_fwd(st, R.c[1].col, 9 * w, c->params + R.c[1].w_off, sb ? R.c[1].wsp : nullptr, R.c[1].z, (int)M, 9 * w, w,
                                                                       epi_stats ? c->rn_part : nullptr, &nb1, c->rn_part_floats); }
            if (rc_) return fail(c, SELD_ERR_INVALID, "resnet50_block: 3x3 convolution's product refused");
            { PROF3(c, "rn_bn_fwd"); rn_bn(c, st, R.c[1], M, p.training, nb1); }
        }
        { PROF3(c, "rn_bn_fwd"); launch_rn_bn_apply(st, R.c[1].z, R.c[1].coef, nullptr, R.y1, M, w, 1); }
        int nb2 = 0;
        { PROF3(c, "rn_products_fwd"); rc_ = launch_rn_product_fwd(st, R.y1, w, c->params + R.c[2].w_off, sb ? R.c[2].wsp : nullptr, R.c[2].z, (int)M, w, 4 * w,
                                                                   epi_stats ? c->rn_part : nullptr, &nb2, c->rn_part_floats); }
        if (rc_) return fail(c, SELD_ERR_INVALID, "resnet50_block: expand convolution's product refused");
        { PROF3(c, "rn_bn_fwd"); rn_bn(c, st, R.c[2], M, p.training, nb2); }
        if (R.proj) {
            if (sc_side) hipStreamWaitEvent(st, c->ev_rn_free[0], 0);
            else {
                int nbs = 0;
                { PROF3(c, "rn_products_fwd"); rc_ = launch_rn_product_fwd(st, X, R.Cin * R.stride_f, c->params + R.sc.w_off, sb ? R.sc.wsp : nullptr, R.sc.z, (int)M, R.Cin, 4 * w,
                                                                           epi_stats ? c->rn_part : nullptr, &nbs, c->rn_part_floats); }
                if (rc_) return fail(c, SELD_ERR_INVALID, "resnet50_block: projection shortcut product refused");
                { PROF3(c, "rn_bn_fwd"); rn_bn(c, st, R.sc, M, p.training, nbs); }
            }
            { PROF3(c, "rn_bn_fwd"); launch_rn_bn_apply2(st, R.c[2].z, R.c[2].coef, R.sc.z, R.sc.coef, R.out, M, 4 * w, p.save ? R.gate : nullptr); }
        } else {
            { PROF3(c, "rn_bn_fwd"); launch_rn_bn_apply(st, R.c[2].z, R.c[2].coef, X, R.out, M, 4 * w, 1, p.save ? R.gate : nullptr); }
        }
        X = R.out;
    }
    if (c->sync_failed) { c->sync_failed = false; return fail(c, SELD_ERR_HIP, "sync_bn all-reduce callback failed"); }
    *feat = X;
    return SELD_OK;
}

static int forward_gru(seld_ctx* c, const FwdPass& p, const float** feat_io) {
    hipStream_t st = c->stream;
    const int B = c->B, S = c->S, rows = B * S;
    const float* feat = *feat_io;
    const int gparts = !c->gram_active ? 0 : (c->gram_parts == 2 && c->gru.size() >= 2 ? 2 : 1);
    int gram_ns = 0;
    for (size_t i = 0; i < c->gru.size(); ++i) {
        GruL& G = c->gru[i];
        if (p.gru_drop) {
            PROF(c, "gru_fwd");
            const float rate = c->arch.gru_dropout;
            for (int d = 0; d < 2; ++d) {
                launch_dropout(st, c->ones, G.imask[d], (int64_t)B * G.in_feat, rate, c->dropout_seed, 96u + 4u * (unsigned)i + d, c->dropout_cur);
                launch_dropout(st, c->ones, G.rmask[d], (int64_t)B * 128, rate, c->dropout_seed, 98u + 4u * (unsigned)i + d, c->dropout_cur);
                launch_mask_rows(st, feat, G.imask[d], G.xm[d], rows, S, G.in_feat, 0);
                if (gru_sb(c, G) && gemm_sb_usable(G.xm[d], G.in_feat, 384, G.in_feat))
                    launch_gemm_sb(st, G.xm[d], nullptr, G.in_feat, c->ksp_fwd[i][d], nullptr, c->params + G.b_off[d], nullptr, G.gx[d], nullptr, 384, rows, 384,
                                   G.in_feat, 0, 0);
                else
                    launch_gemm(st, G.xm[d], G.in_feat, c->params + G.k_off[d], 384, c->params + G.b_off[d], G.gx[d], 384, rows, 384, G.in_feat, 0, 0, 0);
            }
            if (launch_gru_fwd(st, G.gx[0], G.gx[1], c->params + G.u_off[0], c->params + G.u_off[1], c->params + G.b_off[0] + 384,
                               c->params + G.b_off[1] + 384, G.h[0], G.h[1], G.sv[0], G.sv[1], B, S, G.rmask[0], G.rmask[1], G.hm[0], G.hm[1]))
                return fail(c, SELD_ERR_UNSUPPORTED, "gru_fwd (dropout)");
        } else {
        {
            PROF2(c, "gru_inproj_gemm");
            if (gru_sb(c, G) && gemm_sb_usable(feat, G.in_feat, 384, G.in_feat))
                launch_gemm_sb(st, feat, nullptr, G.in_feat, c->ksp_fwd[i][0], c->ksp_fwd[i][1], c->params + G.b_off[0],
                               c->params + G.b_off[1], G.gx[0], G.gx[1], 384, rows, 384, G.in_feat, 0, 1);
            else
                launch_gemm_dual_n(st, feat, G.in_feat, c->params + G.k_off[0], c->params + G.k_off[1], 384, c->params + G.b_off[0],
                                   c->params + G.b_off[1], G.gx[0], G.gx[1], 384, rows, 384, G.in_feat, 0, 0);
        }
        if ((int)i < gparts) fork_side(c);
        {
            PROF(c, "gru_fwd");
            launch_gru_fwd(st, G.gx[0], G.gx[1], c->params + G.u_off[0], c->params + G.u_off[1], c->params + G.b_off[0] + 384,
                           c->params + G.b_off[1] + 384, G.h[0], G.h[1], p.save ? G.sv[0] : nullptr, p.save ? G.sv[1] : nullptr, B, S);
        }
        }
        if ((int)i < gparts && p.gru_drop) fork_side(c);
        if ((int)i < gparts) {
            int ns = 0;
            const int kp = conv_gram_dim(c->conv[0].Cin);
            if (i == 0) gram_ns = 0;
            if (launch_conv_first_gram(c->side, p.x, c->gram_slab + (size_t)gram_ns * kp * kp, &ns, B, c->conv[0].H, c->conv[0].Cin, 1, (int)i, gparts))
                return fail(c, SELD_ERR_UNSUPPORTED, "conv_first_gram");
            gram_ns += ns;
            if ((int)i == gparts - 1) {
                launch_reduce_slabs(c->side, c->gram_slab, gram_ns, (int64_t)kp * kp, c->gram, (int64_t)kp * kp, 0);
                hipEventRecord(c->ev_gram, c->side);
            }
        }
        launch_mul(st, G.h[0], G.h[1], G.out, (int64_t)rows * 128);
        feat = G.out;
    }
    *feat_io = feat;
    return SELD_OK;
}

static int forward_heads(seld_ctx* c, const FwdPass& p, const float* feat, float* sed, float* doa) {
    hipStream_t st = c->stream;
    const int rows = c->B * c->S;
    {
        PROF2(c, "heads_fwd");
        DenseL &S0 = c->heads[0].layers[0], &D0 = c->heads[1].layers[0];
        if (heads_lin(c)) {
            DenseL &S1 = c->heads[0].layers[1], &D1 = c->heads[1].layers[1];
            const int nt = S1.out + D1.out;
            if (launch_gemm_heads(st, feat, S0.in, c->weff, c->weff + (size_t)S0.in * nt, S1.y, D1.y, sed, doa, rows, S1.out, D1.out,
                                  S0.in, c->heads[0].act, c->heads[1].act))
                return fail(c, SELD_ERR_UNSUPPORTED, "gemm_heads");
            return heads_couple(c, doa, rows);
        }
        if (heads_general(c)) {
            for (int hd = 0; hd < 2; ++hd) {
                const float* a = feat;
                Head& Hd = c->heads[hd];
                float* outp = hd == 0 ? sed : doa;
                for (size_t j = 0; j < Hd.layers.size(); ++j) {
                    DenseL& D = Hd.layers[j];
                    const bool lastl = (j + 1 == Hd.layers.size());
                    if (D.ks > 1) { launch_time_expand(st, a, D.xe, c->B, c->S, D.in_base, D.ks); a = D.xe; }
                    launch_gemm_mirror(st, a, D.in, c->params + D.w_off, D.out, c->params + D.b_off, D.y, lastl ? outp : nullptr, D.out,
                                       rows, D.out, D.in, 0, lastl ? Hd.act : Hd.hidden_act);
                    a = D.y;
                    if (!lastl && D.rate > 0.f && p.training) {
                        launch_dropout(st, D.y, D.yd, (int64_t)rows * D.out, D.rate, c->dropout_seed, D.drop_id, c->dropout_cur);
                        a = D.yd;
                    }
                }
            }
            return heads_couple(c, doa, rows);
        }
        const bool merged0 = c->heads[0].layers.size() > 1 && c->heads[1].layers.size() > 1 && S0.in == D0.in && S0.out == D0.out &&
                             c->heads[0].hidden_act == c->heads[1].hidden_act;
        const int hact0 = c->heads[0].hidden_act;
        if (merged0 && heads_sb(c) && gemm_sb_usable(feat, S0.in, S0.out, S0.in))
            launch_gemm_sb(st, feat, nullptr, S0.in, c->h0sp_fwd[0], c->h0sp_fwd[1], c->params + S0.b_off, c->params + D0.b_off, S0.y,
                           D0.y, S0.out, rows, S0.out, S0.in, hact0, 1);
        else if (merged0)
            launch_gemm_dual_n(st, feat, S0.in, c->params + S0.w_off, c->params + D0.w_off, S0.out, c->params + S0.b_off,
                               c->params + D0.b_off, S0.y, D0.y, S0.out, rows, S0.out, S0.in, 0, hact0);
        for (int hd = 0; hd < 2; ++hd) {
            const float* a = feat;
            Head& Hd = c->heads[hd];
            float* outp = hd == 0 ? sed : doa;
            for (size_t j = 0; j < Hd.layers.size(); ++j) {
                DenseL& D = Hd.layers[j];
                const bool lastl = (j + 1 == Hd.layers.size());
                float* y = D.y;
                if (!(merged0 && j == 0))
                    launch_gemm_mirror(st, a, D.in, c->params + D.w_off, D.out, c->params + D.b_off, y, lastl ? outp : nullptr, D.out,
                                       rows, D.out, D.in, 0, lastl ? Hd.act : Hd.hidden_act);
                a = y;
            }
        }
    }
    return heads_couple(c, doa, rows);
}

int forward_impl(seld_ctx* c, const float* x, float* sed, float* doa, int training, bool save) {
    apply_kernel_choices(c);
    c->last_training = training;
    if (training) c->dropout_cur = c->dropout_step++;
    const FwdPass p = {x, training, save, training && c->arch.conv_dropout > 0.f, training && c->arch.gru_dropout > 0.f};
    if (p.gru_drop && !save) return fail(c, SELD_ERR_UNSUPPORTED, "gru_dropout: a training forward without saved gates");
    bool prep_on_side = false, rn_prep_on_side = false;
    const float* feat = nullptr;
    int rc = forward_weight_prep(c, save, &prep_on_side, &rn_prep_on_side);
    if (!rc) rc = forward_conv_blocks(c, p, prep_on_side, &feat);
    if (!rc && c->arch.first_kind == SELD_FIRST_XCEPTION) rc = forward_xception(c, p, &feat);
    if (!rc && c->arch.first_kind == SELD_FIRST_RESNET50) rc = forward_resnet(c, p, rn_prep_on_side, &feat);
    if (!rc) rc = forward_gru(c, p, &feat);
    if (!rc) rc = forward_heads(c, p, feat, sed, doa);
    return rc;
}
```

### seld_amd/csrc/gemm.hip

```cpp
#include "common.h"
#include "prep.h"

#define GT_LDA 65

template <int TRANSB>
__global__ __launch_bounds__(256) void gemm_f32_kernel(const float* __restrict__ A, int lda,
                                                       const float* __restrict__ Bm, int ldb,
                                                       const float* __restrict__ bias, float* __restrict__ C,
                                                       int ldc, int M, int N, int K, int act, int accumulate,
                                                       const float* __restrict__ A1, const float* __restrict__ B1,
                                                       const float* __restrict__ bias1, float* __restrict__ C1, int mode,
                                                       float* __restrict__ M0, float* __restrict__ M1, int nsplit, GemmEpi epi) {
    const int ntx = (N + 63) >> 6;
    const bool second = mode == 1 && (int)blockIdx.x >= ntx;
    if (second) { Bm = B1; bias = bias1; C = C1; }
    constexpr int LDB = TRANSB ? 65 : 64;
    __shared__ __attribute__((aligned(16))) float As[32 * GT_LDA];
    __shared__ __attribute__((aligned(16))) float Bs[32 * LDB];
    const int tid = threadIdx.x, lane = tid & 63, wave = tid >> 6;
    const int hi = lane >> 5, li = lane & 31;
    const int wr = wave >> 1, wc = wave & 1;
    const int m0 = blockIdx.y * 64, n0 = (second ? (int)blockIdx.x - ntx : (int)blockIdx.x) * 64;
    const bool a_vec = ((lda & 3) == 0) && ((K & 3) == 0) && ((reinterpret_cast<uintptr_t>(A) & 15) == 0);
    const bool b_vec = ((ldb & 3) == 0) && (TRANSB ? ((K & 3) == 0) : ((N & 3) == 0)) &&
                       ((reinterpret_cast<uintptr_t>(Bm) & 15) == 0);
    f32x16 acc = zero16(), acc1 = zero16();
    float va[2][4], vb[2][4];
#define GEMM_LOAD(k0_)                                                                                   \
    _Pragma("unroll") for (int u = 0; u < 2; ++u) {                                                      \
        const int idx = tid + 256 * u;                                                                   \
        {                                                                                                \
            const int row = idx >> 3, k4 = (idx & 7) * 4;                                                \
            const int gm = m0 + row, gk = (k0_) + k4;                                                    \
            va[u][0] = va[u][1] = va[u][2] = va[u][3] = 0.f;                                             \
            if (gm < M) {                                                                                \
                const float* p = Ap + (size_t)gm * lda + gk;                                              \
                if (a_vec && gk + 3 < K) {                                                               \
                    const float4 t = *reinterpret_cast<const float4*>(p);                                \
                    va[u][0] = t.x; va[u][1] = t.y; va[u][2] = t.z; va[u][3] = t.w;                      \
                } else {                                                                                 \
                    _Pragma("unroll") for (int j = 0; j < 4; ++j) if (gk + j < K) va[u][j] = p[j];       \
                }                                                                                        \
            }                                                                                            \
        }                                                                                                \
        vb[u][0] = vb[u][1] = vb[u][2] = vb[u][3] = 0.f;                                                 \
        if (TRANSB == 0) {                                                                               \
            const int kk = idx >> 4, n4 = (idx & 15) * 4;                                                \
            const int gk = (k0_) + kk, gn = n0 + n4;                                                     \
            if (gk < K) {                                                                                \
                const float* p = Bp + (size_t)gk * ldb + gn;                                             \
                if (b_vec && gn + 3 < N) {                                                               \
                    const float4 t = *reinterpret_cast<const float4*>(p);                                \
                    vb[u][0] = t.x; vb[u][1] = t.y; vb[u][2] = t.z; vb[u][3] = t.w;                      \
                } else {                                                                                 \
                    _Pragma("unroll") for (int j = 0; j < 4; ++j) if (gn + j < N) vb[u][j] = p[j];       \
                }                                                                                        \
            }                                                                                            \
        } else {                                                                                         \
            const int n = idx >> 3, k4 = (idx & 7) * 4;                                                  \
            const int gn = n0 + n, gk = (k0_) + k4;                                                      \
            if (gn < N) {                                                                                \
                const float* p = Bp + (size_t)gn * ldb + gk;                                             \
                if (b_vec && gk + 3 < K) {                                                               \
                    const float4 t = *reinterpret_cast<const float4*>(p);                                \
                    vb[u][0] = t.x; vb[u][1] = t.y; vb[u][2] = t.z; vb[u][3] = t.w;                      \
                } else {                                                                                 \
                    _Pragma("unroll") for (int j = 0; j < 4; ++j) if (gk + j < K) vb[u][j] = p[j];       \
                }                                                                                        \
            }                                                                                            \
        }                                                                                                \
    }
#define GEMM_COMMIT()                                                                                    \
    _Pragma("unroll") for (int u = 0; u < 2; ++u) {                                                      \
        const int idx = tid + 256 * u;                                                                   \
        {                                                                                                \
            const int row = idx >> 3, k4 = (idx & 7) * 4;                                                \
            _Pragma("unroll") for (int j = 0; j < 4; ++j) As[(k4 + j) * GT_LDA + row] = va[u][j];        \
        }                                                                                                \
        if (TRANSB == 0) {                                                                               \
            const int kk = idx >> 4, n4 = (idx & 15) * 4;                                                \
            *reinterpret_cast<float4*>(&Bs[kk * LDB + n4]) = make_float4(vb[u][0], vb[u][1], vb[u][2], vb[u][3]); \
        } else {                                                                                         \
            const int n = idx >> 3, k4 = (idx & 7) * 4;                                                  \
            _Pragma("unroll") for (int j = 0; j < 4; ++j) Bs[(k4 + j) * LDB + n] = vb[u][j];             \
        }                                                                                                \
    }
    const int nck = (K + 31) >> 5, ng = mode == 2 ? 2 * nck : nck;
#define GEMM_LOADG(g_)                                                                                   \
    {                                                                                                    \
        const int h_ = (g_) >= nck ? 1 : 0;                                                              \
        const float* Ap = h_ ? A1 : A;                                                                   \
        const float* Bp = h_ ? B1 : Bm;                                                                  \
        GEMM_LOAD(((g_) - h_ * nck) * 32)                                                                \
    }
    GEMM_LOADG(0)
    for (int g = 0; g < ng; ++g) {
        GEMM_COMMIT()
        lds_barrier();
        if (g + 1 < ng) GEMM_LOADG(g + 1)
        {
            float ra[4], rb[4];
#pragma unroll
            for (int u = 0; u < 4; ++u) {
                ra[u] = As[(2 * u + hi) * GT_LDA + wr * 32 + li];
                rb[u] = Bs[(2 * u + hi) * LDB + wc * 32 + li];
            }
#pragma unroll
            for (int s = 0; s < 16; ++s) {
                const int u = s & 3;
                __builtin_amdgcn_sched_barrier(0);
                if (s & 1) acc1 = MFMA_F32_32x32x2(ra[u], rb[u], acc1);
                else acc = MFMA_F32_32x32x2(ra[u], rb[u], acc);
                if (s + 4 < 16) {
                    ra[u] = As[(2 * (s + 4) + hi) * GT_LDA + wr * 32 + li];
                    rb[u] = Bs[(2 * (s + 4) + hi) * LDB + wc * 32 + li];
                }
            }
            __builtin_amdgcn_sched_barrier(0);
        }
        lds_barrier();
    }
#undef GEMM_LOADG
#undef GEMM_LOAD
#undef GEMM_COMMIT
    const int col = n0 + wc * 32 + li;
    if (epi.stat_part) {
        float s_ = 0.f, q_ = 0.f;
#pragma unroll
        for (int r = 0; r < 16; ++r) {
            const float v = (m0 + wr * 32 + mfma_row(r, hi) < M) ? acc[r] + acc1[r] : 0.f;
            s_ += v; q_ = fmaf(v, v, q_);
        }
        s_ += __shfl_xor(s_, 32); q_ += __shfl_xor(q_, 32);
        if (hi == 0) { As[(wr * 64 + wc * 32 + li) * 2] = s_; As[(wr * 64 + wc * 32 + li) * 2 + 1] = q_; }
        lds_barrier();
        if (tid < 64) {
            const bool in_ = n0 + tid < N;
            float* pp = epi.stat_part + ((size_t)blockIdx.x * gridDim.y + blockIdx.y) * 128 + tid;
            pp[0] = in_ ? As[tid * 2] + As[(64 + tid) * 2] : 0.f;
            pp[64] = in_ ? As[tid * 2 + 1] + As[(64 + tid) * 2 + 1] : 0.f;
        }
    }
    if ((mode == 0 || mode == 3) && m0 + wr * 32 + 32 <= M && n0 + wc * 32 + 32 <= N && (ldc & 3) == 0 &&
        (reinterpret_cast<uintptr_t>(C) & 15) == 0 && (mode == 0 || (reinterpret_cast<uintptr_t>(C1) & 15) == 0)) {
        const float bv = bias ? bias[col] : 0.f;
        const size_t o0 = (size_t)(m0 + wr * 32 + 4 * hi + (li & 3)) * ldc + n0 + wc * 32 + (li & ~3);
#pragma unroll
        for (int q = 0; q < 4; ++q) {
            float v_[4];
#pragma unroll
            for (int j = 0; j < 4; ++j) {
                v_[j] = (acc[4 * q + j] + acc1[4 * q + j]) + bv;
                if (act == 1) v_[j] = 1.f / (1.f + expf(-v_[j]));
                else if (act == 2) v_[j] = tanhf(v_[j]);
                else if (act == 3) v_[j] = fmaxf(v_[j], 0.f);
            }
            float4 o = quad_transpose4(v_[0], v_[1], v_[2], v_[3], li);
            float4* p = reinterpret_cast<float4*>(C + o0 + (size_t)(8 * q) * ldc);
            if (accumulate) { const float4 c0 = *p; o = make_float4(o.x + c0.x, o.y + c0.y, o.z + c0.z, o.w + c0.w); }
            *p = o;
            if (mode == 3) *reinterpret_cast<float4*>(C1 + o0 + (size_t)(8 * q) * ldc) = o;
        }
        return;
    }
    if (col < N) {
        const float bv = bias ? bias[col] : 0.f;
#pragma unroll
        for (int r = 0; r < 16; ++r) {
            const int row = m0 + wr * 32 + mfma_row(r, hi);
            if (row < M) {
                float v = (acc[r] + acc1[r]) + bv;
                if (mode == 4) {
                    const bool first = col < nsplit;
                    const int a_ = first ? (act & 15) : (act >> 4);
                    if (a_ == 1) v = 1.f / (1.f + expf(-v));
                    else if (a_ == 2) v = tanhf(v);
                    const size_t o_ = first ? (size_t)row * nsplit + col : (size_t)row * (N - nsplit) + (col - nsplit);
                    (first ? C : C1)[o_] = v;
                    float* m_ = first ? M0 : M1;
                    if (m_) m_[o_] = v;
                    continue;
                }
                if (act == 1) v = 1.f / (1.f + expf(-v));
                else if (act == 2) v = tanhf(v);
                else if (act == 3) v = fmaxf(v, 0.f);
                float* p = C + (size_t)row * ldc + col;
                if (accumulate) v += *p;
                *p = v;
                if (mode == 3) C1[(size_t)row * ldc + col] = v;
            }
        }
    }
}

static int gemm_go(hipStream_t st, const float* A, int lda, const float* Bm, int ldb, const float* bias, float* C, int ldc, int M,
                   int N, int K, int transb, int act, int accumulate, const float* A1, const float* B1, const float* bias1, float* C1,
                   int mode, float* M0 = nullptr, float* M1 = nullptr, int nsplit = 0) {
    if (M <= 0 || N <= 0 || K <= 0) return -1;
    if (mode == 2 && (K & 31)) return -2;
    const GemmEpi epi = g_gemm_epi;
    if (epi.stat_part && (bias || act || accumulate || mode)) return -3;
    if (epi.addg) return -3;
// ... 382 lines not shown
```

### seld_amd/csrc/gemm_sb.hip

```cpp
#include "common.h"
#include "prep.h"

typedef __bf16 bf16x8 __attribute__((ext_vector_type(8)));
typedef unsigned u32x4 __attribute__((ext_vector_type(4)));

#define GSB_KC 32
#define GSB_BN 128

__device__ __forceinline__ void gsb_split3_pair(float x0, float x1, unsigned& h, unsigned& m, unsigned& l) {
    const unsigned u0 = __float_as_uint(x0), u1 = __float_as_uint(x1);
    h = __builtin_amdgcn_perm(u1, u0, 0x07060302);
    const float r0 = x0 - __uint_as_float(u0 & 0xffff0000u), r1 = x1 - __uint_as_float(u1 & 0xffff0000u);
    const unsigned v0 = __float_as_uint(r0), v1 = __float_as_uint(r1);
    m = __builtin_amdgcn_perm(v1, v0, 0x07060302);
    const float s0 = r0 - __uint_as_float(v0 & 0xffff0000u), s1 = r1 - __uint_as_float(v1 & 0xffff0000u);
    l = __builtin_amdgcn_perm(__float_as_uint(s1), __float_as_uint(s0), 0x07060302);
}

__device__ __forceinline__ unsigned gsb_rne_pair(float x0, float x1) { return bf16_rne_bits(x0) | (bf16_rne_bits(x1) << 16); }

__global__ __launch_bounds__(256) void gemm_split_b_kernel(GemmSplitJobs jobs) { gemm_split_b_body(jobs, blockIdx.y, blockIdx.x, gridDim.x); }

size_t gemm_sb_split_elems(int K, int N) { return (size_t)3 * K * N; }

int gemm_sb_usable(const void* A, int lda, int N, int K) {
    return (K % GSB_KC) == 0 && (N % GSB_BN) == 0 && (lda & 3) == 0 && (reinterpret_cast<uintptr_t>(A) & 15) == 0;
}

int launch_gemm_split_b(hipStream_t st, int njobs, const float* const* src, unsigned short* const* dst, const int* ldb,
                        const int* transb, const int* K, const int* N) {
    if (njobs <= 0 || njobs > GSB_MAX_JOBS) return -1;
    GemmSplitJobs j;
    j.njobs = njobs;
    j.one = g_mfma_one;
    for (int i = 0; i < njobs; ++i) {
        if (K[i] % GSB_KC) return -2;
        j.src[i] = src[i]; j.dst[i] = dst[i]; j.ldb[i] = ldb[i]; j.transb[i] = transb[i]; j.K[i] = K[i]; j.N[i] = N[i];
    }
    hipLaunchKernelGGL(gemm_split_b_kernel, dim3(144, njobs), dim3(256), 0, st, j);
    return 0;
}

template <int NG, bool ONE = false, bool FOUR = false>
__global__ __launch_bounds__(256, NG == 4 ? 2 : 3) void gemm_sb_kernel(const float* __restrict__ A0, const float* __restrict__ A1, int lda,
                                                         const unsigned short* __restrict__ Bs0,
                                                         const unsigned short* __restrict__ Bs1,
                                                         const float* __restrict__ bias0, const float* __restrict__ bias1,
                                                         float* __restrict__ C0, float* __restrict__ C1, int ldc, int M, int N,
                                                         int K, int act, int mode, int dbg, int accum, GemmEpi epi) {
    __shared__ __attribute__((aligned(16))) unsigned short Bl[2][3 * GSB_BN * GSB_KC];
    const int tid = threadIdx.x, lane = tid & 63, wave = tid >> 6;
    const int kg = lane >> 5, li = lane & 31;
    const int ngrp = N / GSB_BN;
    int grp = blockIdx.x;
    const float* bias = bias0;
    float* C = C0;
    if (mode == 1 && grp >= ngrp) { grp -= ngrp; Bs0 = Bs1; bias = bias1; C = C1; }
    const int n0 = grp * GSB_BN;
    const int m0 = blockIdx.y * 128 + wave * 32;
    const int nck = K / GSB_KC, ng = mode == 2 ? 2 * nck : nck;
    const int arow = min(m0 + li, M - 1);
    const size_t aoff = (size_t)arow * lda + 16 * kg;

    f32x16 acc0 = zero16(), acc1 = zero16(), acc2 = zero16(), acc3 = zero16();
    float4 ca0, ca1, ca2, ca3, na0, na1, na2, na3;
    u32x4 bq0, bq1, bq2, bq3, bq4, bq5;
#define GSB_ISSUE(g_)                                                                                          \
    {                                                                                                          \
        const int h_ = (g_) >= nck ? 1 : 0, gc_ = (g_) - h_ * nck;                                             \
        const float4* ap_ = reinterpret_cast<const float4*>((h_ ? A1 : A0) + aoff + (size_t)gc_ * GSB_KC);     \
        na0 = ap_[0]; na1 = ap_[1]; na2 = ap_[2]; na3 = ap_[3];                                                \
        const u32x4* bp_ = reinterpret_cast<const u32x4*>((h_ ? Bs1 : Bs0) + ((size_t)gc_ * 3 * N + n0) * GSB_KC); \
        const size_t ps_ = (size_t)N * GSB_KC / 8;                             \
        bq0 = bp_[tid]; bq1 = bp_[tid + 256];                                                                  \
        bq2 = bp_[ps_ + tid]; bq3 = bp_[ps_ + tid + 256];                                                      \
        if (!FOUR) { bq4 = bp_[2 * ps_ + tid]; bq5 = bp_[2 * ps_ + tid + 256]; }                               \
    }
#define GSB_COMMIT(buf_)                                                          \
    {                                                                             \
        u32x4* d_ = reinterpret_cast<u32x4*>(Bl[buf_]);                           \
        d_[tid] = bq0; d_[tid + 256] = bq1;                                       \
        d_[512 + tid] = bq2; d_[512 + tid + 256] = bq3;                           \
        if (!FOUR) { d_[1024 + tid] = bq4; d_[1024 + tid + 256] = bq5; }          \
    }
    GSB_ISSUE(0)
    GSB_COMMIT(0)
    ca0 = na0; ca1 = na1; ca2 = na2; ca3 = na3;
    lds_barrier();
    const int swz = (li >> 2) & 3;
    const int boff0 = li * GSB_KC + (((2 * kg) ^ swz) << 3), boff1 = li * GSB_KC + (((2 * kg + 1) ^ swz) << 3);
#define GSB_MFMA(A_, B_, ACC_) ACC_ = __builtin_amdgcn_mfma_f32_32x32x16_bf16(A_, B_, ACC_, 0, 0, 0)
#define GSB_STEP(x0_, x1_, boff_)                                                                     \
    if (ONE) {                                                                                        \
        const u32x4 h_ = {gsb_rne_pair(x0_.x, x0_.y), gsb_rne_pair(x0_.z, x0_.w), gsb_rne_pair(x1_.x, x1_.y), gsb_rne_pair(x1_.z, x1_.w)}; \
        const bf16x8 ah = __builtin_bit_cast(bf16x8, h_);                                             \
        const unsigned short* bb_ = bl + boff_;                                                       \
        const bf16x8 bh0 = *reinterpret_cast<const bf16x8*>(bb_), bh1 = *reinterpret_cast<const bf16x8*>(bb_ + 32 * GSB_KC), \
                     bh2 = *reinterpret_cast<const bf16x8*>(bb_ + 64 * GSB_KC), bh3 = *reinterpret_cast<const bf16x8*>(bb_ + 96 * GSB_KC); \
        GSB_MFMA(ah, bh0, acc0); GSB_MFMA(ah, bh1, acc1); GSB_MFMA(ah, bh2, acc2); GSB_MFMA(ah, bh3, acc3);   \
    } else if (FOUR) {                                                                                \
        unsigned h0_, h1_, h2_, h3_, m0_, m1_, m2_, m3_;                                              \
        split2r_pair(x0_.x, x0_.y, h0_, m0_);                                                         \
        split2r_pair(x0_.z, x0_.w, h1_, m1_);                                                         \
        split2r_pair(x1_.x, x1_.y, h2_, m2_);                                                         \
        split2r_pair(x1_.z, x1_.w, h3_, m3_);                                                         \
        const u32x4 h_ = {h0_, h1_, h2_, h3_}, m_ = {m0_, m1_, m2_, m3_};                             \
        const bf16x8 ah = __builtin_bit_cast(bf16x8, h_), am = __builtin_bit_cast(bf16x8, m_);        \
        const unsigned short* bb_ = bl + boff_;                                                       \
        const bf16x8 bh0 = *reinterpret_cast<const bf16x8*>(bb_), bh1 = *reinterpret_cast<const bf16x8*>(bb_ + 32 * GSB_KC), \
                     bh2 = *reinterpret_cast<const bf16x8*>(bb_ + 64 * GSB_KC), bh3 = *reinterpret_cast<const bf16x8*>(bb_ + 96 * GSB_KC); \
        const unsigned short* bm_ = bb_ + GSB_BN * GSB_KC;                                            \
        const bf16x8 bm0 = *reinterpret_cast<const bf16x8*>(bm_), bm1 = *reinterpret_cast<const bf16x8*>(bm_ + 32 * GSB_KC), \
                     bm2 = *reinterpret_cast<const bf16x8*>(bm_ + 64 * GSB_KC), bm3 = *reinterpret_cast<const bf16x8*>(bm_ + 96 * GSB_KC); \
        GSB_MFMA(ah, bh0, acc0); GSB_MFMA(ah, bh1, acc1); GSB_MFMA(ah, bh2, acc2); GSB_MFMA(ah, bh3, acc3);    \
        GSB_MFMA(ah, bm0, acc0); GSB_MFMA(ah, bm1, acc1); GSB_MFMA(ah, bm2, acc2); GSB_MFMA(ah, bm3, acc3);    \
        GSB_MFMA(am, bh0, acc0); GSB_MFMA(am, bh1, acc1); GSB_MFMA(am, bh2, acc2); GSB_MFMA(am, bh3, acc3);    \
        GSB_MFMA(am, bm0, acc0); GSB_MFMA(am, bm1, acc1); GSB_MFMA(am, bm2, acc2); GSB_MFMA(am, bm3, acc3);    \
    } else                                                                                            \
    {                                                                                                 \
        unsigned h0_, h1_, h2_, h3_, m0_, m1_, m2_, m3_, l0_, l1_, l2_, l3_;                          \
        gsb_split3_pair(x0_.x, x0_.y, h0_, m0_, l0_);                                                 \
        gsb_split3_pair(x0_.z, x0_.w, h1_, m1_, l1_);                                                 \
        gsb_split3_pair(x1_.x, x1_.y, h2_, m2_, l2_);                                                 \
        gsb_split3_pair(x1_.z, x1_.w, h3_, m3_, l3_);                                                 \
        const u32x4 h_ = {h0_, h1_, h2_, h3_}, m_ = {m0_, m1_, m2_, m3_}, l_ = {l0_, l1_, l2_, l3_};  \
        const bf16x8 ah = __builtin_bit_cast(bf16x8, h_), am = __builtin_bit_cast(bf16x8, m_),        \
                     al = __builtin_bit_cast(bf16x8, l_);                                             \
        const unsigned short* bb_ = bl + boff_;                                                       \
        const bf16x8 bh0 = *reinterpret_cast<const bf16x8*>(bb_), bh1 = *reinterpret_cast<const bf16x8*>(bb_ + 32 * GSB_KC), \
                     bh2 = *reinterpret_cast<const bf16x8*>(bb_ + 64 * GSB_KC), bh3 = *reinterpret_cast<const bf16x8*>(bb_ + 96 * GSB_KC); \
        const unsigned short* bm_ = bb_ + GSB_BN * GSB_KC;                                            \
        const bf16x8 bm0 = *reinterpret_cast<const bf16x8*>(bm_), bm1 = *reinterpret_cast<const bf16x8*>(bm_ + 32 * GSB_KC), \
                     bm2 = *reinterpret_cast<const bf16x8*>(bm_ + 64 * GSB_KC), bm3 = *reinterpret_cast<const bf16x8*>(bm_ + 96 * GSB_KC); \
        const unsigned short* bl_ = bm_ + GSB_BN * GSB_KC;                                            \
        const bf16x8 bl0 = *reinterpret_cast<const bf16x8*>(bl_), bl1 = *reinterpret_cast<const bf16x8*>(bl_ + 32 * GSB_KC), \
                     bl2 = *reinterpret_cast<const bf16x8*>(bl_ + 64 * GSB_KC), bl3 = *reinterpret_cast<const bf16x8*>(bl_ + 96 * GSB_KC); \
        GSB_MFMA(ah, bh0, acc0); GSB_MFMA(ah, bh1, acc1); GSB_MFMA(ah, bh2, acc2); GSB_MFMA(ah, bh3, acc3);    \
        GSB_MFMA(ah, bm0, acc0); GSB_MFMA(ah, bm1, acc1); GSB_MFMA(ah, bm2, acc2); GSB_MFMA(ah, bm3, acc3);    \
        GSB_MFMA(am, bh0, acc0); GSB_MFMA(am, bh1, acc1); GSB_MFMA(am, bh2, acc2); GSB_MFMA(am, bh3, acc3);    \
        GSB_MFMA(ah, bl0, acc0); GSB_MFMA(ah, bl1, acc1); GSB_MFMA(ah, bl2, acc2); GSB_MFMA(ah, bl3, acc3);    \
        GSB_MFMA(al, bh0, acc0); GSB_MFMA(al, bh1, acc1); GSB_MFMA(al, bh2, acc2); GSB_MFMA(al, bh3, acc3);    \
        GSB_MFMA(am, bm0, acc0); GSB_MFMA(am, bm1, acc1); GSB_MFMA(am, bm2, acc2); GSB_MFMA(am, bm3, acc3);    \
    }
    if constexpr (NG == 4) {
        float4 pa[4][4];
        u32x4 pb[2][6];
#define GSB_LDA(c_) { const float4* ap_ = reinterpret_cast<const float4*>(A0 + aoff + (size_t)(c_) * GSB_KC); \
                      pa[c_][0] = ap_[0]; pa[c_][1] = ap_[1]; pa[c_][2] = ap_[2]; pa[c_][3] = ap_[3]; }
#define GSB_LDB(c_, set_) { const u32x4* bp_ = reinterpret_cast<const u32x4*>(Bs0 + ((size_t)(c_) * 3 * N + n0) * GSB_KC); \
                            const size_t ps_ = (size_t)N * GSB_KC / 8;                                                       \
                            pb[set_][0] = bp_[tid]; pb[set_][1] = bp_[tid + 256]; pb[set_][2] = bp_[ps_ + tid];              \
                            pb[set_][3] = bp_[ps_ + tid + 256]; if (!FOUR) { pb[set_][4] = bp_[2 * ps_ + tid]; pb[set_][5] = bp_[2 * ps_ + tid + 256]; } }
#define GSB_STB(buf_, set_) { u32x4* d_ = reinterpret_cast<u32x4*>(Bl[buf_]);                                  \
                              d_[tid] = pb[set_][0]; d_[tid + 256] = pb[set_][1]; d_[512 + tid] = pb[set_][2]; \
                              d_[512 + tid + 256] = pb[set_][3]; if (!FOUR) { d_[1024 + tid] = pb[set_][4]; d_[1024 + tid + 256] = pb[set_][5]; } }
        GSB_LDB(1, 1)
        GSB_LDA(1) GSB_LDA(2) GSB_LDA(3)
        pa[0][0] = ca0; pa[0][1] = ca1; pa[0][2] = ca2; pa[0][3] = ca3;
#pragma unroll
        for (int g = 0; g < 4; ++g) {
            if (g + 2 < 4) GSB_LDB(g + 2, g & 1)
            __builtin_amdgcn_sched_barrier(0);
            const unsigned short* bl = Bl[g & 1];
            GSB_STEP(pa[g][0], pa[g][1], boff0)
            GSB_STEP(pa[g][2], pa[g][3], boff1)
            __builtin_amdgcn_sched_barrier(0);
            if (g + 1 < 4) GSB_STB((g + 1) & 1, (g + 1) & 1)
            lds_barrier();
        }
#undef GSB_LDA
#undef GSB_LDB
#undef GSB_STB
    } else
    for (int g = 0; g < ng; ++g) {
        if (!(dbg & 1)) GSB_ISSUE(min(g + 1, ng - 1))
        __builtin_amdgcn_sched_barrier(0);
        const unsigned short* bl = Bl[g & 1];
        GSB_STEP(ca0, ca1, boff0)
        GSB_STEP(ca2, ca3, boff1)
        __builtin_amdgcn_sched_barrier(0);
        GSB_COMMIT((g + 1) & 1)
        ca0 = na0; ca1 = na1; ca2 = na2; ca3 = na3;
        lds_barrier();
    }
#undef GSB_ISSUE
#undef GSB_COMMIT
#undef GSB_STEP
    const float bv0 = bias ? bias[n0 + li] : 0.f, bv1 = bias ? bias[n0 + 32 + li] : 0.f, bv2 = bias ? bias[n0 + 64 + li] : 0.f,
                bv3 = bias ? bias[n0 + 96 + li] : 0.f;
    if (dbg & 2) return;
    const bool full = m0 + 32 <= M;
    float* crow = C + (size_t)(m0 + 4 * kg) * ldc + n0 + li;
    const int rows_left = M - m0 - 4 * kg;
    if (epi.stat_part) {
        float* red = reinterpret_cast<float*>(&Bl[0][0]);
#define GSB_STAT(ACC_, nt_)                                                                  \
        {                                                                                    \
            float s_ = 0.f, q_ = 0.f;                                                        \
            _Pragma("unroll") for (int r = 0; r < 16; ++r) {                                 \
                const int dr = (r & 3) + 8 * (r >> 2);                                       \
                const float v = (full || dr < rows_left) ? ACC_[r] : 0.f;                    \
                s_ += v; q_ = fmaf(v, v, q_);                                                \
            }                                                                                \
            s_ += __shfl_xor(s_, 32); q_ += __shfl_xor(q_, 32);                              \
            if (kg == 0) { red[(wave * 128 + (nt_) * 32 + li) * 2] = s_; red[(wave * 128 + (nt_) * 32 + li) * 2 + 1] = q_; } \
        }
        GSB_STAT(acc0, 0) GSB_STAT(acc1, 1) GSB_STAT(acc2, 2) GSB_STAT(acc3, 3)
#undef GSB_STAT
        lds_barrier();
        if (tid < 128) {
            const float S_ = (red[tid * 2] + red[(128 + tid) * 2]) + (red[(256 + tid) * 2] + red[(384 + tid) * 2]);
            const float Q_ = (red[tid * 2 + 1] + red[(128 + tid) * 2 + 1]) + (red[(256 + tid) * 2 + 1] + red[(384 + tid) * 2 + 1]);
            const int gc = n0 + tid;
            float* pp = epi.stat_part + ((size_t)(gc >> 6) * gridDim.y + blockIdx.y) * 128 + (gc & 63);
            pp[0] = S_; pp[64] = Q_;
        }
    }
    if (epi.addg) {
#define GSB_ADDG(ACC_, nt_)                                                                  \
        _Pragma("unroll") for (int r = 0; r < 16; ++r) {                                     \
            const int dr = (r & 3) + 8 * (r >> 2);                                           \
            if (full || dr < rows_left) {                                                    \
                const size_t e_ = (size_t)(m0 + 4 * kg + dr) * ldc + n0 + (nt_) * 32 + li;   \
                const unsigned g_ = epi.gate4[e_ >> 2];                                      \
                ACC_[r] += ((g_ >> (e_ & 3)) & 1u) ? epi.addg[e_] : 0.f;                     \
            }                                                                                \
        }
        GSB_ADDG(acc0, 0) GSB_ADDG(acc1, 1) GSB_ADDG(acc2, 2) GSB_ADDG(acc3, 3)
#undef GSB_ADDG
    }
#define GSB_STORE(ACC_, nt_, BV_)                                                            \
    _Pragma("unroll") for (int r = 0; r < 16; ++r) {                                         \
        const int dr = (r & 3) + 8 * (r >> 2);                                               \
        float v = ACC_[r] + BV_;                                                             \
        if (act == 1) v = 1.f / (1.f + expf(-v));                                            \
        else if (act == 2) v = tanhf(v);                                                     \
        else if (act == 3) v = fmaxf(v, 0.f);                                                \
        if (full || dr < rows_left) {                                                        \
            if (accum) v += crow[(size_t)dr * ldc + (nt_) * 32];                             \
            crow[(size_t)dr * ldc + (nt_) * 32] = v;                                         \
        }                                                                                    \
    }
    if (act == 0 && full && !accum) {
#define GSB_STORE_PLAIN(ACC_, nt_, BV_)                                                      \
    _Pragma("unroll") for (int r = 0; r < 16; ++r) crow[(size_t)((r & 3) + 8 * (r >> 2)) * ldc + (nt_) * 32] = ACC_[r] + BV_;
        GSB_STORE_PLAIN(acc0, 0, bv0) GSB_STORE_PLAIN(acc1, 1, bv1) GSB_STORE_PLAIN(acc2, 2, bv2) GSB_STORE_PLAIN(acc3, 3, bv3)
#undef GSB_STORE_PLAIN
    } else {
        GSB_STORE(acc0, 0, bv0) GSB_STORE(acc1, 1, bv1) GSB_STORE(acc2, 2, bv2) GSB_STORE(acc3, 3, bv3)
    }
#undef GSB_STORE
}

template <int NG, bool CONV = false, bool ONE = false, bool FOUR = false>
__global__ __launch_bounds__(1024) void gemm_sb16_kernel(const float* __restrict__ A0, const float* __restrict__ A1, int lda,
                                                         const unsigned short* __restrict__ Bs0,
                                                         const unsigned short* __restrict__ Bs1,
                                                         const float* __restrict__ bias0, const float* __restrict__ bias1,
                                                         float* __restrict__ C0, float* __restrict__ C1, int ldc, int M, int N,
                                                         int K, int act, int mode, int accum, int cvs, int cvH, int cvW, GemmEpi epi) {
    __shared__ __attribute__((aligned(16))) unsigned short Al[2][3 * 128 * GSB_KC];
    __shared__ __attribute__((aligned(16))) unsigned short Bl[2][3 * GSB_BN * GSB_KC];
    const int tid = threadIdx.x, lane = tid & 63, wave = tid >> 6;
    const int kg = lane >> 5, li = lane & 31, wr = wave >> 2, wc = wave & 3;
    const int ngrp = N / GSB_BN;
    int grp = blockIdx.x;
    const float* bias = bias0;
    float* C = C0;
    if (mode == 1 && grp >= ngrp) { grp -= ngrp; Bs0 = Bs1; bias = bias1; C = C1; }
    const int n0 = grp * GSB_BN, m0 = blockIdx.y * 128;
// ... 216 lines not shown

template <bool FOUR>
__global__ __launch_bounds__(512) void gemm_sbp_kernel(const float* __restrict__ A, int lda, const unsigned short* __restrict__ Bs0,
                                                       const unsigned short* __restrict__ Bs1, const float* __restrict__ bias0,
                                                       const float* __restrict__ bias1, float* __restrict__ C0, float* __restrict__ C1, int ldc, int M,
                                                       int N, int ngroups, int dbg) {
    constexpr int NPL = FOUR ? 2 : 3;
    extern __shared__ __attribute__((aligned(16))) unsigned short sbp_smem[];
    const int tid = threadIdx.x, lane = tid & 63, wave = tid >> 6;
    const int kg = lane >> 5, li = lane & 31;
    const int ngrp = N / GSB_BN;
    int grp = blockIdx.x % ngroups;
    const int wig = blockIdx.x / ngroups, wpg = gridDim.x / ngroups;
    const unsigned short* Bs = Bs0;
    const float* bias = bias0;
    float* C = C0;
    if (grp >= ngrp) { grp -= ngrp; Bs = Bs1; bias = bias1; C = C1; }
    const int n0 = grp * GSB_BN;
    if (!(dbg & 8))
#pragma unroll
    for (int j = 0; j < 4 * NPL; ++j) {
        const int c = j / NPL, p = j - c * NPL;
        reinterpret_cast<u32x4*>(sbp_smem)[(c * 3 + p) * 512 + tid] =
            reinterpret_cast<const u32x4*>(Bs + ((size_t)(c * 3 + p) * N + n0) * GSB_KC)[tid];
    }
    const int ntile = (M + 31) / 32, slots = wpg * 8;
    int t = wave * wpg + wig;
    float4 pa[4][4];
#define SBP_LDA(tile_)                                                                                            \
    {                                                                                                             \
        const float4* ap_ = reinterpret_cast<const float4*>(A + (size_t)min((tile_) * 32 + li, M - 1) * lda + 16 * kg); \
        _Pragma("unroll") for (int c_ = 0; c_ < 4; ++c_) {                                                        \
            pa[c_][0] = ap_[8 * c_]; pa[c_][1] = ap_[8 * c_ + 1]; pa[c_][2] = ap_[8 * c_ + 2]; pa[c_][3] = ap_[8 * c_ + 3]; \
        }                                                                                                         \
    }
    if (t < ntile) SBP_LDA(t)
#undef SBP_LDA
    const float4 bv0 = bias ? *reinterpret_cast<const float4*>(bias + n0 + (li & ~3)) : make_float4(0.f, 0.f, 0.f, 0.f),
                 bv1 = bias ? *reinterpret_cast<const float4*>(bias + n0 + 32 + (li & ~3)) : make_float4(0.f, 0.f, 0.f, 0.f),
                 bv2 = bias ? *reinterpret_cast<const float4*>(bias + n0 + 64 + (li & ~3)) : make_float4(0.f, 0.f, 0.f, 0.f),
                 bv3 = bias ? *reinterpret_cast<const float4*>(bias + n0 + 96 + (li & ~3)) : make_float4(0.f, 0.f, 0.f, 0.f);
    __syncthreads();
    const int swz = (li >> 2) & 3;
    const int bo0 = li * GSB_KC + (((2 * kg) ^ swz) << 3), bo1 = li * GSB_KC + (((2 * kg + 1) ^ swz) << 3);
    for (; t < ntile; t += slots) {
        const int m0 = t * 32;
        const int tn = t + slots < ntile ? t + slots : t;
        const float4* an = reinterpret_cast<const float4*>(A + (size_t)min(tn * 32 + li, M - 1) * lda + 16 * kg);
        f32x16 acc0 = zero16(), acc1 = zero16(), acc2 = zero16(), acc3 = zero16();
        int o0 = bo0, o1 = bo1;
        asm volatile("" : "+v"(o0), "+v"(o1));
        const unsigned short *b0 = sbp_smem + o0, *b1 = sbp_smem + o1;
#pragma unroll
        for (int g = 0; g < 4; ++g) {
            if (!(dbg & 1)) sbp_step<FOUR>(pa[g][0], pa[g][1], b0 + g * 3 * 4096, acc0, acc1, acc2, acc3);
            __builtin_amdgcn_sched_barrier(0);
            if (!(dbg & 1)) sbp_step<FOUR>(pa[g][2], pa[g][3], b1 + g * 3 * 4096, acc0, acc1, acc2, acc3);
            __builtin_amdgcn_sched_barrier(0);
            if (!(dbg & 4)) { pa[g][0] = an[8 * g]; pa[g][1] = an[8 * g + 1]; pa[g][2] = an[8 * g + 2]; pa[g][3] = an[8 * g + 3]; }
            __builtin_amdgcn_sched_barrier(0);
        }
        if (dbg & 2) continue;
        float* crow = C + (size_t)(m0 + 4 * kg + (li & 3)) * ldc + n0 + (li & ~3);
        const int rows_left = M - m0 - 4 * kg - (li & 3);
        const bool full = m0 + 32 <= M;
#define SBP_STORE(ACC_, nt_, BV_, GUARD_)                                                                         \
        _Pragma("unroll") for (int q = 0; q < 4; ++q) {                                                           \
            float4 o = quad_transpose4(ACC_[4 * q], ACC_[4 * q + 1], ACC_[4 * q + 2], ACC_[4 * q + 3], li);      \
            o.x += BV_.x; o.y += BV_.y; o.z += BV_.z; o.w += BV_.w;                                               \
            if (!(GUARD_) || 8 * q < rows_left) *reinterpret_cast<float4*>(crow + (size_t)(8 * q) * ldc + (nt_) * 32) = o; \
        }
        if (full) { SBP_STORE(acc0, 0, bv0, false) SBP_STORE(acc1, 1, bv1, false) SBP_STORE(acc2, 2, bv2, false) SBP_STORE(acc3, 3, bv3, false) }
        else { SBP_STORE(acc0, 0, bv0, true) SBP_STORE(acc1, 1, bv1, true) SBP_STORE(acc2, 2, bv2, true) SBP_STORE(acc3, 3, bv3, true) }
#undef SBP_STORE
    }
}

int g_gsb_dbg = 0;
thread_local GemmEpi g_gemm_epi;
int gemm_epi_row_blocks(int M, int split_bf16) { return split_bf16 ? (M + 127) / 128 : (M + 63) / 64; }
thread_local int g_gsb_four_now = 0;
int launch_gemm_sb(hipStream_t st, const float* A0, const float* A1, int lda, const unsigned short* Bs0, const unsigned short* Bs1,
                   const float* bias0, const float* bias1, float* C0, float* C1, int ldc, int M, int N, int K, int act, int mode,
                   int accum, int conv_C, int conv_H, int conv_W) {
    int cvs = 0;
    if (conv_C) {
        while ((1 << cvs) < conv_C) ++cvs;
        if ((1 << cvs) != conv_C || conv_C < 32 || K != 9 * conv_C || mode != 0 || conv_H <= 0 || conv_W <= 0 || M % (conv_H * conv_W)) return -1;
        lda = conv_C;
    }
    if (M <= 0 || N <= 0 || K <= 0 || !gemm_sb_usable(A0, lda, N, K)) return -1;
    if (mode == 2 && !gemm_sb_usable(A1, lda, N, K)) return -1;
    const GemmEpi epi = g_gemm_epi;
    if (epi.stat_part && (bias0 || act || mode || accum)) return -3;
    if (epi.addg && (!epi.gate4 || (ldc & 3) || mode)) return -3;
    dim3 grid(N / GSB_BN * (mode == 1 ? 2 : 1), (M + 127) / 128);
    const bool wide = grid.x >= 2;
    if (cvs ? false : (g_gsb_dbg & 4) ? true : (g_gsb_dbg & 8) ? false : wide) {
#define GSB_GO(NG_) { if (g_mfma_one) hipLaunchKernelGGL((gemm_sb_kernel<NG_, true>), grid, dim3(256), 0, st, A0, A1, lda, Bs0, Bs1, bias0, bias1, C0, C1, ldc, M, N, K, act, \
                                       mode, g_gsb_dbg & 3, accum, epi);                                                                                            \
                      else if (g_gsb_four_now) hipLaunchKernelGGL((gemm_sb_kernel<NG_, false, true>), grid, dim3(256), 0, st, A0, A1, lda, Bs0, Bs1, bias0, bias1, C0, C1, ldc, M, N, K, act, \
                                       mode, g_gsb_dbg & 3, accum, epi);                                                                                            \
                      else hipLaunchKernelGGL((gemm_sb_kernel<NG_, false>), grid, dim3(256), 0, st, A0, A1, lda, Bs0, Bs1, bias0, bias1, C0, C1, ldc, M, N, K, act, \
                                       mode, g_gsb_dbg & 3, accum, epi); }
        if (K == 128 && mode != 2 && !act && !accum && !epi.stat_part && !epi.addg && !g_mfma_one && (g_gsb_dbg & 64) && !(g_gsb_dbg & 3) &&  (int)grid.x <= 128 &&
            !(ldc & 3) && !(reinterpret_cast<uintptr_t>(C0) & 15) && !(reinterpret_cast<uintptr_t>(C1) & 15)) {
            const int ngroups = (int)grid.x, wpg = 256 / ngroups;
            const int need = ((M + 31) / 32 + 7) / 8;
            const int w = wpg < need ? wpg : need;
            const size_t smem = (size_t)4 * 3 * 4096 * sizeof(unsigned short);
            if (g_gsb_four_now) {
                hipFuncSetAttribute(reinterpret_cast<const void*>(gemm_sbp_kernel<true>), hipFuncAttributeMaxDynamicSharedMemorySize, (int)smem);
                hipLaunchKernelGGL((gemm_sbp_kernel<true>), dim3(ngroups * w), dim3(512), smem, st, A0, lda, Bs0, Bs1, bias0, bias1, C0, C1, ldc, M, N, ngroups, g_gsb_dbg >> 8);
            } else {
                hipFuncSetAttribute(reinterpret_cast<const void*>(gemm_sbp_kernel<false>), hipFuncAttributeMaxDynamicSharedMemorySize, (int)smem);
                hipLaunchKernelGGL((gemm_sbp_kernel<false>), dim3(ngroups * w), dim3(512), smem, st, A0, lda, Bs0, Bs1, bias0, bias1, C0, C1, ldc, M, N, ngroups, g_gsb_dbg >> 8);
            }
            return 0;
        }
        if (K == 128 && mode != 2 && !(g_gsb_dbg & 32)) GSB_GO(4)
        else GSB_GO(0)
#undef GSB_GO
    } else {
        const int ng = K / GSB_KC * (mode == 2 ? 2 : 1);
#define G16_GO(NG_, CV_) { if (g_gsb_four_now) hipLaunchKernelGGL((gemm_sb16_kernel<NG_, CV_, false, true>), grid, dim3(1024), 0, st, A0, A1, lda, Bs0, Bs1, bias0, bias1, C0, C1, ldc, M, N, K, act, mode, accum, cvs, conv_H, conv_W, epi); \
                           else hipLaunchKernelGGL((gemm_sb16_kernel<NG_, CV_>), grid, dim3(1024), 0, st, A0, A1, lda, Bs0, Bs1, bias0, bias1, C0, C1, ldc, M, N, K, act, mode, accum, cvs, conv_H, conv_W, epi); }
#define G16_GO1(NG_) hipLaunchKernelGGL((gemm_sb16_kernel<NG_, false, true>), grid, dim3(1024), 0, st, A0, A1, lda, Bs0, Bs1, bias0, bias1, C0, C1, ldc, M, N, K, act, mode, accum, cvs, conv_H, conv_W, epi)
        if (g_mfma_one && !cvs && !(g_gsb_dbg & 16) && (ng == 24 || ng == 4)) { if (ng == 24) G16_GO1(24); else G16_GO1(4); return 0; }
        if (g_mfma_one && !cvs && ng != 36 && ng != 16 && ng != 12 && ng != 8) { G16_GO1(0); return 0; }
        if (cvs) { if (ng == 36) G16_GO(36, true) else if (ng == 72) G16_GO(72, true) else G16_GO(0, true) }
        else if (g_gsb_dbg & 16) G16_GO(0, false)
        else if (ng == 36) G16_GO(36, false)
        else if (ng == 24) G16_GO(24, false)
        else if (ng == 16) G16_GO(16, false)
        else if (ng == 12) G16_GO(12, false)
        else if (ng == 8) G16_GO(8, false)
        else if (ng == 4) G16_GO(4, false)
        else G16_GO(0, false)
#undef G16_GO
#undef G16_GO1
    }
    return 0;
}
```

### seld_amd/csrc/loss_adam.hip

```cpp
#include "common.h"

#define BCE_EPS 1e-7f

__global__ __launch_bounds__(1024) void reduce_rows_kernel(const float* __restrict__ in, int rows, int ncol,
                                                           double* __restrict__ out) {
    __shared__ double red[1024];
    for (int c = 0; c < ncol; ++c) {
        double s = 0.0;
        for (int r = threadIdx.x; r < rows; r += 1024) s += (double)in[(size_t)r * ncol + c];
        red[threadIdx.x] = s;
        __syncthreads();
        for (int w = 512; w > 0; w >>= 1) {
            if ((int)threadIdx.x < w) red[threadIdx.x] += red[threadIdx.x + w];
            __syncthreads();
        }
        if (threadIdx.x == 0) out[c] = red[0];
        __syncthreads();
    }
}

__global__ __launch_bounds__(256) void mmse_mask_rows_kernel(const float* __restrict__ y_doa, float* __restrict__ rowsum,
                                                             int rows, int nc) {
    const int r = blockIdx.x * 256 + threadIdx.x;
    if (r >= rows) return;
    const float* y = y_doa + (size_t)r * 3 * nc;
    float s = 0.f;
    for (int c = 0; c < nc; ++c) {
        const float a = y[c], b = y[nc + c], d = y[2 * nc + c];
        s += 3.f * rintf(a * a + b * b + d * d);
    }
    rowsum[r] = s;
}

__global__ void den_store_kernel(const double* __restrict__ sums, float* __restrict__ den) { den[0] = (float)sums[0]; }

int loss_scratch_floats(int rows) { return rows * 2 + 64; }

int launch_mmse_den(hipStream_t st, const float* y_doa, float* den, float* scratch, int rows, int nc) {
    double* sums = reinterpret_cast<double*>(scratch + (size_t)rows * 2);
    hipLaunchKernelGGL(mmse_mask_rows_kernel, dim3((rows + 255) / 256), dim3(256), 0, st, y_doa, scratch, rows, nc);
    hipLaunchKernelGGL(reduce_rows_kernel, dim3(1), dim3(1024), 0, st, scratch, rows, 1, sums);
    hipLaunchKernelGGL(den_store_kernel, dim3(1), dim3(1), 0, st, sums, den);
    return 0;
}

__device__ __forceinline__ float loss_quad_sum(float v) {
    v += __int_as_float(__builtin_amdgcn_update_dpp(0, __float_as_int(v), 0xB1 , 0xF, 0xF, true));
    v += __int_as_float(__builtin_amdgcn_update_dpp(0, __float_as_int(v), 0x4E , 0xF, 0xF, true));
    return v;
}

__global__ __launch_bounds__(256) void losses_kernel(const float* __restrict__ sed, const float* __restrict__ doa,
                                                     const float* __restrict__ y_sed, const float* __restrict__ y_doa,
                                                     int doa_loss, float coef_sed, float w_doa,
                                                     const float* __restrict__ den_dev, float* __restrict__ dloss_rows,
                                                     float* __restrict__ dsed_pre, float* __restrict__ ddoa_pre,
                                                     double* __restrict__ blockpart, int rows, int nc, int ld_sed, int ld_doa) {
    __shared__ float rs[64][2];
    const int q = threadIdx.x & 3, rl = threadIdx.x >> 2;
    const int r = min(blockIdx.x * 64 + rl, rows - 1);
    const bool live = blockIdx.x * 64 + rl < rows;
    const float* p = sed + (size_t)r * nc;
    const float* ys = y_sed + (size_t)r * nc;
    float bsum = 0.f;
    for (int c = q; c < nc; c += 4) {
        const float pv = p[c], y = ys[c];
        const float pc = fminf(fmaxf(pv, BCE_EPS), 1.f - BCE_EPS);
        bsum += -(y * logf(pc + BCE_EPS) + (1.f - y) * logf(1.f - pc + BCE_EPS));
        if (dsed_pre && live) {
            const bool pass = (pv >= BCE_EPS) && (pv <= 1.f - BCE_EPS);
            const float dldp = pass ? -(y / (pc + BCE_EPS) - (1.f - y) / (1.f - pc + BCE_EPS)) : 0.f;
            dsed_pre[(size_t)r * ld_sed + c] = coef_sed * dldp * pv * (1.f - pv);
        }
    }
    const float* d = doa + (size_t)r * 3 * nc;
    const float* yd = y_doa + (size_t)r * 3 * nc;
    float dsum = 0.f;
    if (doa_loss != 1) {
        const float inv = 1.f / (float)(3 * nc);
        for (int k = q; k < 3 * nc; k += 4) {
            const float pk = d[k], yk = yd[k];
            float term, dldp;
            if (doa_loss == 0) {
                const float e = yk - pk;
                term = e * e;
                dldp = -2.f * e;
            } else if (doa_loss == 2) {
                const float e = pk - yk;
                term = fabsf(e);
                dldp = e > 0.f ? 1.f : (e < 0.f ? -1.f : 0.f);
            } else {
                const float lp = logf(fmaxf(pk, BCE_EPS) + 1.f), ly = logf(fmaxf(yk, BCE_EPS) + 1.f);
                const float e = lp - ly;
                term = e * e;
                const float pass = pk > BCE_EPS ? 1.f : (pk == BCE_EPS ? 0.5f : 0.f);
                dldp = 2.f * e * pass / (fmaxf(pk, BCE_EPS) + 1.f);
            }
            dsum += term;
            if (ddoa_pre && live) ddoa_pre[(size_t)r * ld_doa + k] = w_doa * (dldp * inv) * (1.f - pk * pk);
        }
        dsum = loss_quad_sum(dsum) * inv;
        if (dloss_rows && live && q == 0) dloss_rows[r] = dsum;
    } else {
        const float den = den_dev[0];
        for (int c = q; c < nc; c += 4) {
            const float a = yd[c], b = yd[nc + c], e3 = yd[2 * nc + c];
            const float m = rintf(a * a + b * b + e3 * e3);
            for (int k = 0; k < 3; ++k) {
                const int i = k * nc + c;
                const float e = yd[i] - d[i];
                dsum += e * e * m;
                if (ddoa_pre && live) ddoa_pre[(size_t)r * ld_doa + i] = w_doa * (-2.f * e * m / den) * (1.f - d[i] * d[i]);
            }
        }
        dsum = loss_quad_sum(dsum);
    }
    bsum = loss_quad_sum(bsum);
    if (q == 0) { rs[rl][0] = live ? bsum : 0.f; rs[rl][1] = live ? dsum : 0.f; }
    __syncthreads();
    if (threadIdx.x < 2) {
        double s = 0.0;
        for (int i = 0; i < 64; ++i) s += (double)rs[i][threadIdx.x];
        blockpart[(size_t)blockIdx.x * 2 + threadIdx.x] = s;
    }
}

__global__ __launch_bounds__(64) void losses_finalize_kernel(const double* __restrict__ blockpart, int nblocks, int doa_loss, double n_sed,
                                                             const float* __restrict__ den_dev, float* __restrict__ sloss,
                                                             float* __restrict__ dloss) {
    double s0 = 0.0, s1 = 0.0;
    for (int i = threadIdx.x; i < nblocks; i += 64) { s0 += blockpart[2 * i]; s1 += blockpart[2 * i + 1]; }
#pragma unroll
    for (int w = 32; w > 0; w >>= 1) { s0 += __shfl_xor(s0, w); s1 += __shfl_xor(s1, w); }
    if (threadIdx.x) return;
    if (sloss) sloss[0] = (float)(s0 / n_sed);
    if (doa_loss == 1 && dloss) dloss[0] = (float)(s1 / (double)den_dev[0]);
}

int launch_losses_finalize(hipStream_t st, int doa_loss, const float* den_dev, float* sloss, float* dloss, float* scratch, int B, int S,
                           int nc);
int launch_losses(hipStream_t st, const float* sed, const float* doa, const float* y_sed, const float* y_doa,
                  int doa_loss, float w_sed, float w_doa, float sed_grad_scale, const float* den_dev,
                  float* sloss, float* dloss, float* dsed_pre, float* ddoa_pre, float* scratch, int B, int S, int nc, int ld_sed,
                  int ld_doa, int defer_finalize) {
    if (ld_sed <= 0) ld_sed = nc;
    if (ld_doa <= 0) ld_doa = 3 * nc;
    const int rows = B * S;
    const float coef_sed = w_sed * sed_grad_scale * (doa_loss != 1 ? (float)rows : 1.f) / ((float)rows * (float)nc);
    double* blockpart = reinterpret_cast<double*>(scratch);
    const int nblocks = (rows + 63) / 64;
    hipLaunchKernelGGL(losses_kernel, dim3(nblocks), dim3(256), 0, st, sed, doa, y_sed, y_doa, doa_loss, coef_sed, w_doa, den_dev,
                       doa_loss != 1 ? dloss : nullptr, dsed_pre, ddoa_pre, blockpart, rows, nc, ld_sed, ld_doa);
    if (!defer_finalize) launch_losses_finalize(st, doa_loss, den_dev, sloss, dloss, scratch, B, S, nc);
    return 0;
}

int launch_losses_finalize(hipStream_t st, int doa_loss, const float* den_dev, float* sloss, float* dloss, float* scratch, int B, int S,
                           int nc) {
    const int rows = B * S, nblocks = (rows + 63) / 64;
    hipLaunchKernelGGL(losses_finalize_kernel, dim3(1), dim3(64), 0, st, reinterpret_cast<const double*>(scratch), nblocks, doa_loss,
                       (double)rows * nc, den_dev, sloss, dloss);
    return 0;
}

__global__ __launch_bounds__(256) void adam_kernel(float* __restrict__ theta, const float* __restrict__ g,
                                                   float* __restrict__ m, float* __restrict__ v, int64_t n, float lr_t,
                                                   float b1, float b2, float eps) {
    const int64_t i = (int64_t)blockIdx.x * 256 + threadIdx.x;
    if (i >= n) return;
    const float gi = g[i];
    const float mi = b1 * m[i] + (1.f - b1) * gi;
    const float vi = b2 * v[i] + (1.f - b2) * gi * gi;
    m[i] = mi;
    v[i] = vi;
    theta[i] = theta[i] - lr_t * mi / (sqrtf(vi) + eps);
}

int launch_adam(hipStream_t st, float* theta, const float* g, float* m, float* v, int64_t n, float lr_t,
                float beta1, float beta2, float eps) {
    hipLaunchKernelGGL(adam_kernel, dim3((unsigned)((n + 255) / 256)), dim3(256), 0, st, theta, g, m, v, n, lr_t, beta1,
                       beta2, eps);
    return 0;
}

__global__ __launch_bounds__(256) void agc_kernel(const float* __restrict__ theta, float* __restrict__ g, int rows, int cols) {
    const int c = blockIdx.x * 256 + threadIdx.x;
    if (c >= cols) return;
    float pn = 0.f, gn = 0.f;
    for (int r = 0; r < rows; ++r) {
        const float p = theta[(size_t)r * cols + c], gg = g[(size_t)r * cols + c];
        pn += p * p;
        gn += gg * gg;
    }
    pn = sqrtf(pn);
    gn = sqrtf(gn);
    const float max_norm = fmaxf(pn, 1e-3f) * 0.01f;
    if (!(gn < max_norm)) {
        const float sc = max_norm / fmaxf(gn, 1e-6f);
        for (int r = 0; r < rows; ++r) g[(size_t)r * cols + c] *= sc;
    }
}

int launch_agc(hipStream_t st, const float* theta, float* g, int64_t off, int rank, const int64_t* shape, float* scratch) {
    (void)scratch;
    int rows = 1, cols = 1;
    if (rank <= 1) { rows = (int)shape[0]; cols = 1; }
    else if (rank == 2) { rows = (int)shape[0]; cols = (int)shape[1]; }
    else if (rank == 3) { rows = (int)shape[0]; cols = (int)(shape[1] * shape[2]); }
    else { rows = (int)(shape[0] * shape[1] * shape[2]); cols = (int)shape[3]; }
    hipLaunchKernelGGL(agc_kernel, dim3((cols + 255) / 256), dim3(256), 0, st, theta + off, g + off, rows, cols);
    return 0;
}

__global__ __launch_bounds__(256) void act_bwd_kernel(const float4* __restrict__ y, float4* __restrict__ dy, int64_t n4, int act) {
    const int64_t i = (int64_t)blockIdx.x * 256 + threadIdx.x;
    if (i >= n4) return;
    const float4 v = y[i];
    float4 d = dy[i];
    if (act == 1) { d.x *= v.x * (1.f - v.x); d.y *= v.y * (1.f - v.y); d.z *= v.z * (1.f - v.z); d.w *= v.w * (1.f - v.w); }
    else if (act == 2) { d.x *= 1.f - v.x * v.x; d.y *= 1.f - v.y * v.y; d.z *= 1.f - v.z * v.z; d.w *= 1.f - v.w * v.w; }
    else if (act == 3) { d.x = v.x > 0.f ? d.x : 0.f; d.y = v.y > 0.f ? d.y : 0.f; d.z = v.z > 0.f ? d.z : 0.f; d.w = v.w > 0.f ? d.w : 0.f; }
    dy[i] = d;
}
int launch_act_bwd(hipStream_t st, const float* y, float* dy, int64_t n, int act) {
    if (n & 3) return -1;
    const int64_t n4 = n >> 2;
    hipLaunchKernelGGL(act_bwd_kernel, dim3((unsigned)((n4 + 255) / 256)), dim3(256), 0, st, reinterpret_cast<const float4*>(y),
                       reinterpret_cast<float4*>(dy), n4, act);
    return 0;
}

// ... 128 lines not shown
```

Before: 12710 clips/s.

## Fuse GRU gate multiply into next in-proj GEMM and fuse heads with losses

Adds a fused heads+loss step kernel that runs the final GRU gate multiply, the linear SED/DOA heads, the BCE/MSE losses and the head-gradient computation in one launch, and skips the separate loss and backward-heads launches when it ran. Separately, the elementwise GRU gate multiply between layers is folded into the next layer's split-bf16 input-projection GEMM, which multiplies its A operand on the fly and writes the product for later use. Both aim to remove kernel launches and round-trips of row-sized activations through global memory. In exchange the code adds conditional paths with many eligibility checks and extra register pressure in the GEMM kernel.

After: 12820 clips/s, median of 6. No clear change (+0.8%).

```diff
diff --git a/seld_amd/csrc/api.hip b/seld_amd/csrc/api.hip
--- a/seld_amd/csrc/api.hip
+++ b/seld_amd/csrc/api.hip
@@ -463,6 +463,8 @@
     if (!strcmp(key, "conv64_split_bf16")) { c->conv64_split_bf16 = value != 0; return SELD_OK; }
     if (!strcmp(key, "gemm_split_bf16")) { c->gemm_split_bf16 = value != 0; return SELD_OK; }
     if (!strcmp(key, "heads_fused")) { c->heads_fused = value != 0; return SELD_OK; }
+    if (!strcmp(key, "heads_step")) { c->heads_step = value != 0; return SELD_OK; }
+    if (!strcmp(key, "gru_mul_fused")) { c->gru_mul_fused = value != 0; return SELD_OK; }
     if (!strcmp(key, "dropout_seed")) { c->dropout_seed = 0x5e1d5e1d00000000ull ^ (uint64_t)(unsigned)value; return SELD_OK; }
     if (!strcmp(key, "dropout_step")) { c->dropout_step = (unsigned)value; return SELD_OK; }
     if (!strcmp(key, "conv1_split_bf16")) { c->conv1_split_bf16 = value != 0; return SELD_OK; }
@@ -614,9 +616,10 @@
                        float* sed, float* doa, float* sloss, float* dloss) {
     if (!c || !x || !y_sed || !y_doa || !cfg) return SELD_ERR_INVALID;
     HIPCHK(c, hipSetDevice(c->device));
-    int rc = forward_impl(c, x, sed, doa, 1, true);
+    const StepLosses sl = {y_sed, y_doa, cfg, sloss, dloss};
+    int rc = forward_impl(c, x, sed, doa, 1, true, &sl);
     if (rc) return rc;
-    rc = run_losses(c, y_sed, y_doa, cfg, sloss, dloss, true, true);
+    if (!c->heads_step_done) rc = run_losses(c, y_sed, y_doa, cfg, sloss, dloss, true, true);
     if (rc) return rc;
     return backward_impl(c, x);
 }
diff --git a/seld_amd/csrc/backward.hip b/seld_amd/csrc/backward.hip
--- a/seld_amd/csrc/backward.hip
+++ b/seld_amd/csrc/backward.hip
@@ -74,6 +74,7 @@
 }
 
 static int backward_heads(seld_ctx* c) {
+    if (c->heads_step_done) { c->heads_step_done = false; return SELD_OK; }
     hipStream_t st = c->stream;
     const int rows = c->B * c->S;
     GruL& Glast = c->gru.back();
diff --git a/seld_amd/csrc/common.h b/seld_amd/csrc/common.h
--- a/seld_amd/csrc/common.h
+++ b/seld_amd/csrc/common.h
@@ -258,7 +258,8 @@
 int launch_gemm_sb(hipStream_t st, const float* A0, const float* A1, int lda, const unsigned short* Bs0, const unsigned short* Bs1,
                    const float* bias0, const float* bias1, float* C0, float* C1, int ldc, int M, int N, int K, int act, int mode,
                    int accum = 0,
-                   int conv_C = 0, int conv_H = 0, int conv_W = 0);
+                   int conv_C = 0, int conv_H = 0, int conv_W = 0,
+                   const float* Amul = nullptr, float* Pout = nullptr);
 int launch_gemm_tn(hipStream_t st, const float* A, int lda, const float* Bm, int ldb, float* slab, int* nslab,
                    int M, int K1, int N, int S, int shift, int want_bias, int max_splits = 0, int chunk_rows = 32);
 int gemm_tn_sb_usable(const void* A, int lda, const void* Bm, int ldb, int K1, int N);
@@ -318,6 +319,18 @@
                   int ld_doa = 0, int defer_finalize = 0);
 int launch_losses_finalize(hipStream_t st, int doa_loss, const float* den_dev, float* sloss, float* dloss, float* scratch, int B, int S,
                            int nc);
+float losses_coef_sed(float w_sed, float sed_grad_scale, int doa_loss, int rows, int nc);
+struct HeadsStep {
+    const float *hf, *hb; float* out;
+    const float* weff;
+    float *y0, *y1, *m0, *m1;
+    const float *ys, *yd;
+    int doa_loss; float coef_sed, w_doa;
+    float *dloss_rows, *dy_all; double* blockpart; float* dfeat;
+    int rows, nc, n0, nt, act0, act1;
+};
+int heads_step_usable(const HeadsStep& a);
+int launch_heads_step(hipStream_t st, const HeadsStep& a);
 int loss_scratch_floats(int rows);
 int launch_adam(hipStream_t st, float* theta, const float* g, float* m, float* v, int64_t n, float lr_t,
                 float beta1, float beta2, float eps);
diff --git a/seld_amd/csrc/ctx.h b/seld_amd/csrc/ctx.h
--- a/seld_amd/csrc/ctx.h
+++ b/seld_amd/csrc/ctx.h
@@ -119,6 +119,9 @@
     int conv1_pool_fused = 1;
     int heads_fused = 1;
     float *weff = nullptr, *dy_all = nullptr, *headF = nullptr;
+    int heads_step = 1;
+    bool heads_step_done = false;
+    int gru_mul_fused = 1;
     int rn_split_bf16 = 1;
     int gemm_split_bf16 = 1;
     unsigned short* gsplit = nullptr;
@@ -217,7 +220,8 @@
 int rn_c1_width(const RnBlock& R);
 bool rn_c1_direct(const RnBlock& R);
 
-int forward_impl(seld_ctx* c, const float* x, float* sed, float* doa, int training, bool save);
+struct StepLosses { const float *y_sed, *y_doa; const seld_loss_cfg* cfg; float *sloss, *dloss; };
+int forward_impl(seld_ctx* c, const float* x, float* sed, float* doa, int training, bool save, const StepLosses* losses = nullptr);
 int backward_impl(seld_ctx* c, const float* x);
 
 int v2_tables_create(seld_ctx* c);
diff --git a/seld_amd/csrc/forward.hip b/seld_amd/csrc/forward.hip
--- a/seld_amd/csrc/forward.hip
+++ b/seld_amd/csrc/forward.hip
@@ -109,7 +109,17 @@
     int training;
     bool save;
     bool conv_drop, gru_drop;
+    const StepLosses* losses;
+    bool heads_step;
 };
+
+static bool heads_step_ok(const seld_ctx* c, const StepLosses* l, bool gru_drop) {
+    if (!l || !c->heads_step || !heads_lin(c) || c->arch.output_coupling || gru_drop || c->gru.empty()) return false;
+    const int dl = l->cfg->doa_loss;
+    if (dl != SELD_DOA_MSE && dl != SELD_DOA_MAE && dl != SELD_DOA_MSLE) return false;
+    const int nc = c->arch.n_classes;
+    return c->heads[0].layers[0].in == 128 && c->heads[0].layers[1].out == nc && c->heads[1].layers[1].out == 3 * nc;
+}
 
 static int forward_weight_prep(seld_ctx* c, bool save, bool* prep_on_side, bool* rn_prep_on_side) {
     hipStream_t st = c->stream;
@@ -360,6 +370,8 @@
     const float* feat = *feat_io;
     const int gparts = !c->gram_active ? 0 : (c->gram_parts == 2 && c->gru.size() >= 2 ? 2 : 1);
     int gram_ns = 0;
+    const float* mul_b = nullptr;
+    float* mul_out = nullptr;
     for (size_t i = 0; i < c->gru.size(); ++i) {
         GruL& G = c->gru[i];
         if (p.gru_drop) {
@@ -381,12 +393,19 @@
         } else {
         {
             PROF2(c, "gru_inproj_gemm");
+            if (mul_b && launch_gemm_sb(st, feat, nullptr, G.in_feat, c->ksp_fwd[i][0], c->ksp_fwd[i][1], c->params + G.b_off[0], c->params + G.b_off[1], G.gx[0],
+                                        G.gx[1], 384, rows, 384, G.in_feat, 0, 1, 0, 0, 0, 0, mul_b, mul_out) == 0) {
+                feat = mul_out;
+                mul_b = nullptr;
+            } else {
+            if (mul_b) { launch_mul(st, feat, mul_b, mul_out, (int64_t)rows * 128); feat = mul_out; mul_b = nullptr; }
             if (gru_sb(c, G) && gemm_sb_usable(feat, G.in_feat, 384, G.in_feat))
                 launch_gemm_sb(st, feat, nullptr, G.in_feat, c->ksp_fwd[i][0], c->ksp_fwd[i][1], c->params + G.b_off[0],
                                c->params + G.b_off[1], G.gx[0], G.gx[1], 384, rows, 384, G.in_feat, 0, 1);
             else
                 launch_gemm_dual_n(st, feat, G.in_feat, c->params + G.k_off[0], c->params + G.k_off[1], 384, c->params + G.b_off[0],
                                    c->params + G.b_off[1], G.gx[0], G.gx[1], 384, rows, 384, G.in_feat, 0, 0);
+            }
         }
         if ((int)i < gparts) fork_side(c);
         {
@@ -408,7 +427,12 @@
                 hipEventRecord(c->ev_gram, c->side);
             }
         }
-        launch_mul(st, G.h[0], G.h[1], G.out, (int64_t)rows * 128);
+        const bool last = i + 1 == c->gru.size();
+        if (!last && c->gru_mul_fused && !p.gru_drop && gru_sb(c, c->gru[i + 1]) && c->gru[i + 1].in_feat == 128) {
+            feat = G.h[0]; mul_b = G.h[1]; mul_out = G.out;
+            continue;
+        }
+        if (!(p.heads_step && last)) launch_mul(st, G.h[0], G.h[1], G.out, (int64_t)rows * 128);
         feat = G.out;
     }
     *feat_io = feat;
@@ -424,6 +448,20 @@
         if (heads_lin(c)) {
             DenseL &S1 = c->heads[0].layers[1], &D1 = c->heads[1].layers[1];
             const int nt = S1.out + D1.out;
+            if (p.heads_step) {
+                const StepLosses& l = *p.losses;
+                const GruL& G = c->gru.back();
+                float* sl = l.sloss ? l.sloss : c->loss_out;
+                float* dl = l.dloss ? l.dloss : c->loss_out + 4;
+                const HeadsStep a = {G.h[0], G.h[1], G.out, c->weff, S1.y, D1.y, sed, doa, l.y_sed, l.y_doa, l.cfg->doa_loss,
+                                     losses_coef_sed(l.cfg->w_sed, l.cfg->sed_grad_scale, l.cfg->doa_loss, rows, c->arch.n_classes), l.cfg->w_doa,
+                                     dl, c->dy_all, reinterpret_cast<double*>(c->loss_scratch), c->feat_grad, rows, c->arch.n_classes, S1.out, nt,
+                                     c->heads[0].act, c->heads[1].act};
+                if (launch_heads_step(st, a)) return fail(c, SELD_ERR_UNSUPPORTED, "heads_step");
+                c->fin_sl = sl; c->fin_dl = dl; c->fin_doa_loss = l.cfg->doa_loss;
+                c->heads_step_done = true;
+                return check_launch(c, "heads_step");
+            }
             if (launch_gemm_heads(st, feat, S0.in, c->weff, c->weff + (size_t)S0.in * nt, S1.y, D1.y, sed, doa, rows, S1.out, D1.out,
                                   S0.in, c->heads[0].act, c->heads[1].act))
                 return fail(c, SELD_ERR_UNSUPPORTED, "gemm_heads");
@@ -476,11 +514,13 @@
     return heads_couple(c, doa, rows);
 }
 
-int forward_impl(seld_ctx* c, const float* x, float* sed, float* doa, int training, bool save) {
+int forward_impl(seld_ctx* c, const float* x, float* sed, float* doa, int training, bool save, const StepLosses* losses) {
     apply_kernel_choices(c);
     c->last_training = training;
+    c->heads_step_done = false;
     if (training) c->dropout_cur = c->dropout_step++;
-    const FwdPass p = {x, training, save, training && c->arch.conv_dropout > 0.f, training && c->arch.gru_dropout > 0.f};
+    const bool gru_drop = training && c->arch.gru_dropout > 0.f;
+    const FwdPass p = {x, training, save, training && c->arch.conv_dropout > 0.f, gru_drop, losses, save && heads_step_ok(c, losses, gru_drop)};
     if (p.gru_drop && !save) return fail(c, SELD_ERR_UNSUPPORTED, "gru_dropout: a training forward without saved gates");
     bool prep_on_side = false, rn_prep_on_side = false;
     const float* feat = nullptr;
diff --git a/seld_amd/csrc/gemm.hip b/seld_amd/csrc/gemm.hip
--- a/seld_amd/csrc/gemm.hip
+++ b/seld_amd/csrc/gemm.hip
@@ -1,7 +1,6 @@
 #include "common.h"
 #include "prep.h"
-
-#define GT_LDA 65
+#include "gemm_tile.h"
 
 template <int TRANSB>
 __global__ __launch_bounds__(256) void gemm_f32_kernel(const float* __restrict__ A, int lda,
@@ -98,26 +97,7 @@
         GEMM_COMMIT()
         lds_barrier();
         if (g + 1 < ng) GEMM_LOADG(g + 1)
-        {
-            float ra[4], rb[4];
-#pragma unroll
-            for (int u = 0; u < 4; ++u) {
-                ra[u] = As[(2 * u + hi) * GT_LDA + wr * 32 + li];
-                rb[u] = Bs[(2 * u + hi) * LDB + wc * 32 + li];
-            }
-#pragma unroll
-            for (int s = 0; s < 16; ++s) {
-                const int u = s & 3;
-                __builtin_amdgcn_sched_barrier(0);
-                if (s & 1) acc1 = MFMA_F32_32x32x2(ra[u], rb[u], acc1);
-                else acc = MFMA_F32_32x32x2(ra[u], rb[u], acc);
-                if (s + 4 < 16) {
-                    ra[u] = As[(2 * (s + 4) + hi) * GT_LDA + wr * 32 + li];
-                    rb[u] = Bs[(2 * (s + 4) + hi) * LDB + wc * 32 + li];
-                }
-            }
-            __builtin_amdgcn_sched_barrier(0);
-        }
+        gemm_f32_chunk<GT_LDA, LDB>(As + wr * 32 + li, Bs + wc * 32 + li, hi, acc, acc1);
         lds_barrier();
     }
 #undef GEMM_LOADG
diff --git a/seld_amd/csrc/gemm_sb.hip b/seld_amd/csrc/gemm_sb.hip
--- a/seld_amd/csrc/gemm_sb.hip
+++ b/seld_amd/csrc/gemm_sb.hip
@@ -15,6 +15,11 @@
     m = __builtin_amdgcn_perm(v1, v0, 0x07060302);
     const float s0 = r0 - __uint_as_float(v0 & 0xffff0000u), s1 = r1 - __uint_as_float(v1 & 0xffff0000u);
     l = __builtin_amdgcn_perm(__float_as_uint(s1), __float_as_uint(s0), 0x07060302);
+}
+
+__device__ __forceinline__ float4 gsb_mul4(const float4& x, const float4& y) {
+#pragma clang fp contract(off)
+    return make_float4(x.x * y.x, x.y * y.y, x.z * y.z, x.w * y.w);
 }
 
 __device__ __forceinline__ unsigned gsb_rne_pair(float x0, float x1) { return bf16_rne_bits(x0) | (bf16_rne_bits(x1) << 16); }
@@ -41,13 +46,13 @@
     return 0;
 }
 
-template <int NG, bool ONE = false, bool FOUR = false>
+template <int NG, bool ONE = false, bool FOUR = false, bool MUL = false>
 __global__ __launch_bounds__(256, NG == 4 ? 2 : 3) void gemm_sb_kernel(const float* __restrict__ A0, const float* __restrict__ A1, int lda,
                                                          const unsigned short* __restrict__ Bs0,
                                                          const unsigned short* __restrict__ Bs1,
                                                          const float* __restrict__ bias0, const float* __restrict__ bias1,
                                                          float* __restrict__ C0, float* __restrict__ C1, int ldc, int M, int N,
-                                                         int K, int act, int mode, int dbg, int accum, GemmEpi epi) {
+                                                         int K, int act, int mode, int dbg, int accum, GemmEpi epi, float* __restrict__ P) {
     __shared__ __attribute__((aligned(16))) unsigned short Bl[2][3 * GSB_BN * GSB_KC];
     const int tid = threadIdx.x, lane = tid & 63, wave = tid >> 6;
     const int kg = lane >> 5, li = lane & 31;
@@ -83,6 +88,10 @@
         d_[512 + tid] = bq2; d_[512 + tid + 256] = bq3;                           \
         if (!FOUR) { d_[1024 + tid] = bq4; d_[1024 + tid + 256] = bq5; }          \
     }
+    float4 pm[2][4];
+#define GSB_LDM(c_) { const float4* mp_ = reinterpret_cast<const float4*>(A1 + aoff + (size_t)(c_) * GSB_KC); \
+                      pm[(c_) & 1][0] = mp_[0]; pm[(c_) & 1][1] = mp_[1]; pm[(c_) & 1][2] = mp_[2]; pm[(c_) & 1][3] = mp_[3]; }
+    if (MUL) GSB_LDM(0)
     GSB_ISSUE(0)
     GSB_COMMIT(0)
     ca0 = na0; ca1 = na1; ca2 = na2; ca3 = na3;
@@ -155,11 +164,24 @@
                               d_[tid] = pb[set_][0]; d_[tid + 256] = pb[set_][1]; d_[512 + tid] = pb[set_][2]; \
                               d_[512 + tid + 256] = pb[set_][3]; if (!FOUR) { d_[1024 + tid] = pb[set_][4]; d_[1024 + tid + 256] = pb[set_][5]; } }
         GSB_LDB(1, 1)
-        GSB_LDA(1) GSB_LDA(2) GSB_LDA(3)
+        if (MUL) { GSB_LDA(1) GSB_LDM(1) }
+        else { GSB_LDA(1) GSB_LDA(2) GSB_LDA(3) }
         pa[0][0] = ca0; pa[0][1] = ca1; pa[0][2] = ca2; pa[0][3] = ca3;
+        const bool pstore = MUL && blockIdx.x == 0 && m0 + li < M;
 #pragma unroll
         for (int g = 0; g < 4; ++g) {
             if (g + 2 < 4) GSB_LDB(g + 2, g & 1)
+            if (MUL) {
+#pragma unroll
+                for (int j = 0; j < 4; ++j) {
+                    pa[g][j] = gsb_mul4(pa[g][j], pm[g & 1][j]);
+                }
+                if (g + 2 < 4) { GSB_LDA(g + 2) GSB_LDM(g + 2) }
+                if (pstore) {
+                    float4* pp_ = reinterpret_cast<float4*>(P + aoff + (size_t)g * GSB_KC);
+                    pp_[0] = pa[g][0]; pp_[1] = pa[g][1]; pp_[2] = pa[g][2]; pp_[3] = pa[g][3];
+                }
+            }
             __builtin_amdgcn_sched_barrier(0);
             const unsigned short* bl = Bl[g & 1];
             GSB_STEP(pa[g][0], pa[g][1], boff0)
@@ -186,6 +208,7 @@
 #undef GSB_ISSUE
 #undef GSB_COMMIT
 #undef GSB_STEP
+#undef GSB_LDM
     const float bv0 = bias ? bias[n0 + li] : 0.f, bv1 = bias ? bias[n0 + 32 + li] : 0.f, bv2 = bias ? bias[n0 + 64 + li] : 0.f,
                 bv3 = bias ? bias[n0 + 96 + li] : 0.f;
     if (dbg & 2) return;
@@ -568,8 +591,17 @@
 thread_local int g_gsb_four_now = 0;
 int launch_gemm_sb(hipStream_t st, const float* A0, const float* A1, int lda, const unsigned short* Bs0, const unsigned short* Bs1,
                    const float* bias0, const float* bias1, float* C0, float* C1, int ldc, int M, int N, int K, int act, int mode,
-                   int accum, int conv_C, int conv_H, int conv_W) {
+                   int accum, int conv_C, int conv_H, int conv_W, const float* Amul, float* Pout) {
     int cvs = 0;
+    if (Amul) {
+        if (conv_C || M <= 0 || K != 128 || mode == 2 || N / GSB_BN * (mode == 1 ? 2 : 1) < 2 || !gemm_sb_usable(A0, lda, N, K) || !gemm_sb_usable(Amul, lda, N, K) ||
+            !Pout || (reinterpret_cast<uintptr_t>(Pout) & 15) || g_mfma_one || g_gsb_four_now || g_gsb_dbg || g_gemm_epi.stat_part || g_gemm_epi.addg)
+            return -4;
+        dim3 grid(N / GSB_BN * (mode == 1 ? 2 : 1), (M + 127) / 128);
+        hipLaunchKernelGGL((gemm_sb_kernel<4, false, false, true>), grid, dim3(256), 0, st, A0, Amul, lda, Bs0, Bs1, bias0, bias1, C0, C1, ldc, M, N, K, act, mode, 0, accum,
+                           g_gemm_epi, Pout);
+        return 0;
+    }
     if (conv_C) {
         while ((1 << cvs) < conv_C) ++cvs;
         if ((1 << cvs) != conv_C || conv_C < 32 || K != 9 * conv_C || mode != 0 || conv_H <= 0 || conv_W <= 0 || M % (conv_H * conv_W)) return -1;
@@ -584,11 +616,11 @@
     const bool wide = grid.x >= 2;
     if (cvs ? false : (g_gsb_dbg & 4) ? true : (g_gsb_dbg & 8) ? false : wide) {
 #define GSB_GO(NG_) { if (g_mfma_one) hipLaunchKernelGGL((gemm_sb_kernel<NG_, true>), grid, dim3(256), 0, st, A0, A1, lda, Bs0, Bs1, bias0, bias1, C0, C1, ldc, M, N, K, act, \
-                                       mode, g_gsb_dbg & 3, accum, epi);                                                                                            \
+                                       mode, g_gsb_dbg & 3, accum, epi, nullptr);                                                                                            \
                       else if (g_gsb_four_now) hipLaunchKernelGGL((gemm_sb_kernel<NG_, false, true>), grid, dim3(256), 0, st, A0, A1, lda, Bs0, Bs1, bias0, bias1, C0, C1, ldc, M, N, K, act, \
-                                       mode, g_gsb_dbg & 3, accum, epi);                                                                                            \
+                                       mode, g_gsb_dbg & 3, accum, epi, nullptr);                                                                                            \
                       else hipLaunchKernelGGL((gemm_sb_kernel<NG_, false>), grid, dim3(256), 0, st, A0, A1, lda, Bs0, Bs1, bias0, bias1, C0, C1, ldc, M, N, K, act, \
-                                       mode, g_gsb_dbg & 3, accum, epi); }
+                                       mode, g_gsb_dbg & 3, accum, epi, nullptr); }
         if (K == 128 && mode != 2 && !act && !accum && !epi.stat_part && !epi.addg && !g_mfma_one && (g_gsb_dbg & 64) && !(g_gsb_dbg & 3) &&  (int)grid.x <= 128 &&
             !(ldc & 3) && !(reinterpret_cast<uintptr_t>(C0) & 15) && !(reinterpret_cast<uintptr_t>(C1) & 15)) {
             const int ngroups = (int)grid.x, wpg = 256 / ngroups;
diff --git a/seld_amd/csrc/gemm_tile.h b/seld_amd/csrc/gemm_tile.h
--- /dev/null
+++ b/seld_amd/csrc/gemm_tile.h
@@ -0,0 +1,26 @@
+#pragma once
+#include "common.h"
+
+#define GT_LDA 65
+
+template <int AK, int BK>
+__device__ __forceinline__ void gemm_f32_chunk(const float* a, const float* b, int hi, f32x16& acc, f32x16& acc1) {
+    float ra[4], rb[4];
+#pragma unroll
+    for (int u = 0; u < 4; ++u) {
+        ra[u] = a[(2 * u + hi) * AK];
+        rb[u] = b[(2 * u + hi) * BK];
+    }
+#pragma unroll
+    for (int s = 0; s < 16; ++s) {
+        const int u = s & 3;
+        __builtin_amdgcn_sched_barrier(0);
+        if (s & 1) acc1 = MFMA_F32_32x32x2(ra[u], rb[u], acc1);
+        else acc = MFMA_F32_32x32x2(ra[u], rb[u], acc);
+        if (s + 4 < 16) {
+            ra[u] = a[(2 * (s + 4) + hi) * AK];
+            rb[u] = b[(2 * (s + 4) + hi) * BK];
+        }
+    }
+    __builtin_amdgcn_sched_barrier(0);
+}
diff --git a/seld_amd/csrc/heads_step.hip b/seld_amd/csrc/heads_step.hip
--- /dev/null
+++ b/seld_amd/csrc/heads_step.hip
@@ -0,0 +1,121 @@
+#include "common.h"
+#include "gemm_tile.h"
+#include "loss_rows.h"
+
+#define HS_K 128
+
+__global__ __launch_bounds__(256) void heads_step_kernel(HeadsStep a) {
+    extern __shared__ __attribute__((aligned(16))) float hs_smem[];
+    float* Af = hs_smem;
+    float* Wl = hs_smem + HS_K * GT_LDA;
+    float (*rs)[2] = reinterpret_cast<float (*)[2]>(hs_smem + 2 * HS_K * GT_LDA);
+    float* Ys = Af;
+    float* dyT = Af + 64 * GT_LDA;
+    const int tid = threadIdx.x, lane = tid & 63, wave = tid >> 6;
+    const int hi = lane >> 5, li = lane & 31;
+    const int wr = wave >> 1, wc = wave & 1;
+    const int m0 = blockIdx.x * 64, M = a.rows, nt = a.nt;
+    float4 f[8], b[8];
+#pragma unroll
+    for (int u = 0; u < 8; ++u) {
+        const int idx = tid + 256 * u, row = idx >> 5, c4 = (idx & 31) * 4;
+        f[u] = b[u] = make_float4(0.f, 0.f, 0.f, 0.f);
+        if (m0 + row < M) {
+            f[u] = *reinterpret_cast<const float4*>(a.hf + (size_t)(m0 + row) * HS_K + c4);
+            b[u] = *reinterpret_cast<const float4*>(a.hb + (size_t)(m0 + row) * HS_K + c4);
+        }
+    }
+    const int col = wc * 32 + li;
+    const float bv = col < nt ? a.weff[(size_t)HS_K * nt + col] : 0.f;
+#pragma unroll
+    for (int u = 0; u < 8; ++u) {
+        const int idx = tid + 256 * u, k = idx >> 4, c4 = (idx & 15) * 4;
+        const float4 w = c4 < nt ? *reinterpret_cast<const float4*>(a.weff + (size_t)k * nt + c4) : make_float4(0.f, 0.f, 0.f, 0.f);
+        float* d = Wl + k * GT_LDA + c4;
+        d[0] = w.x; d[1] = w.y; d[2] = w.z; d[3] = w.w;
+    }
+#pragma unroll
+    for (int u = 0; u < 8; ++u) {
+        const int idx = tid + 256 * u, row = idx >> 5, c4 = (idx & 31) * 4;
+        const float4 p = make_float4(f[u].x * b[u].x, f[u].y * b[u].y, f[u].z * b[u].z, f[u].w * b[u].w);
+        if (m0 + row < M) *reinterpret_cast<float4*>(a.out + (size_t)(m0 + row) * HS_K + c4) = p;
+        Af[(c4 + 0) * GT_LDA + row] = p.x; Af[(c4 + 1) * GT_LDA + row] = p.y;
+        Af[(c4 + 2) * GT_LDA + row] = p.z; Af[(c4 + 3) * GT_LDA + row] = p.w;
+    }
+    lds_barrier();
+    f32x16 acc = zero16(), acc1 = zero16();
+#pragma unroll
+    for (int g = 0; g < HS_K / 32; ++g)
+        gemm_f32_chunk<GT_LDA, GT_LDA>(Af + 32 * g * GT_LDA + wr * 32 + li, Wl + 32 * g * GT_LDA + wc * 32 + li, hi, acc, acc1);
+    lds_barrier();
+    if (col < nt) {
+        const bool first = col < a.n0;
+        const int a_ = first ? a.act0 : a.act1;
+        const int w_ = first ? a.n0 : nt - a.n0, c_ = first ? col : col - a.n0;
+        float* y_ = first ? a.y0 : a.y1;
+        float* m_ = first ? a.m0 : a.m1;
+#pragma unroll
+        for (int r = 0; r < 16; ++r) {
+            const int rl = wr * 32 + mfma_row(r, hi);
+            float v = (acc[r] + acc1[r]) + bv;
+            if (a_ == 1) v = 1.f / (1.f + expf(-v));
+            else if (a_ == 2) v = tanhf(v);
+            Ys[rl * GT_LDA + col] = v;
+            if (m0 + rl < M) {
+                const size_t o_ = (size_t)(m0 + rl) * w_ + c_;
+                y_[o_] = v;
+                if (m_) m_[o_] = v;
+            }
+        }
+    }
+    for (int i = nt * GT_LDA + tid; i < 64 * GT_LDA; i += 256) dyT[i] = 0.f;
+    lds_barrier();
+    {
+        const int q = tid & 3, rl = tid >> 2;
+        const bool live = m0 + rl < M;
+        const int rc = live ? rl : M - 1 - m0;
+        const size_t r = (size_t)m0 + rc;
+        float bsum, dsum;
+        loss_row_terms(Ys + rc * GT_LDA, Ys + rc * GT_LDA + a.n0, a.ys + r * a.nc, a.yd + r * 3 * a.nc, a.doa_loss, a.coef_sed, a.w_doa, nullptr,
+                       a.dloss_rows ? a.dloss_rows + r : nullptr, a.dy_all + r * nt, a.dy_all + r * nt + a.n0, dyT + rl, dyT + a.n0 * GT_LDA + rl,
+                       a.nc, q, live, bsum, dsum);
+        loss_block_sums(rs, bsum, dsum, q, rl, live, a.blockpart);
+    }
+    const bool full = m0 + wr * 32 + 32 <= M;
+#pragma unroll
+    for (int j = 0; j < HS_K / 64; ++j) {
+        acc = zero16(); acc1 = zero16();
+#pragma unroll
+        for (int g = 0; g < 2; ++g)
+            gemm_f32_chunk<GT_LDA, 1>(dyT + 32 * g * GT_LDA + wr * 32 + li, Wl + (64 * j + wc * 32 + li) * GT_LDA + 32 * g, hi, acc, acc1);
+        const float bz = 0.f;
+        if (full) {
+            float* o0 = a.dfeat + (size_t)(m0 + wr * 32 + 4 * hi + (li & 3)) * HS_K + 64 * j + wc * 32 + (li & ~3);
+#pragma unroll
+            for (int q = 0; q < 4; ++q)
+                *reinterpret_cast<float4*>(o0 + (size_t)(8 * q) * HS_K) =
+                    quad_transpose4((acc[4 * q] + acc1[4 * q]) + bz, (acc[4 * q + 1] + acc1[4 * q + 1]) + bz, (acc[4 * q + 2] + acc1[4 * q + 2]) + bz,
+                                    (acc[4 * q + 3] + acc1[4 * q + 3]) + bz, li);
+        } else {
+#pragma unroll
+            for (int r = 0; r < 16; ++r) {
+                const int row = m0 + wr * 32 + mfma_row(r, hi);
+                if (row < M) a.dfeat[(size_t)row * HS_K + 64 * j + wc * 32 + li] = (acc[r] + acc1[r]) + bz;
+            }
+        }
+    }
+}
+
+int heads_step_usable(const HeadsStep& a) {
+    const auto al16 = [](const void* p) { return (reinterpret_cast<uintptr_t>(p) & 15) == 0; };
+    return a.rows > 0 && a.nc > 0 && a.n0 == a.nc && a.nt == 4 * a.nc && a.nt <= 64 && a.doa_loss != 1 && al16(a.hf) && al16(a.hb) && al16(a.out) &&
+           al16(a.weff) && al16(a.dfeat);
+}
+
+int launch_heads_step(hipStream_t st, const HeadsStep& a) {
+    if (!heads_step_usable(a)) return -1;
+    const size_t smem = ((size_t)2 * HS_K * GT_LDA + 128) * sizeof(float);
+    if (hipFuncSetAttribute(reinterpret_cast<const void*>(heads_step_kernel), hipFuncAttributeMaxDynamicSharedMemorySize, (int)smem) != hipSuccess) return -2;
+    hipLaunchKernelGGL(heads_step_kernel, dim3((a.rows + 63) / 64), dim3(256), smem, st, a);
+    return 0;
+}
diff --git a/seld_amd/csrc/loss_adam.hip b/seld_amd/csrc/loss_adam.hip
--- a/seld_amd/csrc/loss_adam.hip
+++ b/seld_amd/csrc/loss_adam.hip
@@ -1,6 +1,5 @@
 #include "common.h"
-
-#define BCE_EPS 1e-7f
+#include "loss_rows.h"
 
 __global__ __launch_bounds__(1024) void reduce_rows_kernel(const float* __restrict__ in, int rows, int ncol,
                                                            double* __restrict__ out) {
@@ -44,12 +43,6 @@
     return 0;
 }
 
-__device__ __forceinline__ float loss_quad_sum(float v) {
-    v += __int_as_float(__builtin_amdgcn_update_dpp(0, __float_as_int(v), 0xB1 , 0xF, 0xF, true));
-    v += __int_as_float(__builtin_amdgcn_update_dpp(0, __float_as_int(v), 0x4E , 0xF, 0xF, true));
-    return v;
-}
-
 __global__ __launch_bounds__(256) void losses_kernel(const float* __restrict__ sed, const float* __restrict__ doa,
                                                      const float* __restrict__ y_sed, const float* __restrict__ y_doa,
                                                      int doa_loss, float coef_sed, float w_doa,
@@ -60,69 +53,11 @@
     const int q = threadIdx.x & 3, rl = threadIdx.x >> 2;
     const int r = min(blockIdx.x * 64 + rl, rows - 1);
     const bool live = blockIdx.x * 64 + rl < rows;
-    const float* p = sed + (size_t)r * nc;
-    const float* ys = y_sed + (size_t)r * nc;
-    float bsum = 0.f;
-    for (int c = q; c < nc; c += 4) {
-        const float pv = p[c], y = ys[c];
-        const float pc = fminf(fmaxf(pv, BCE_EPS), 1.f - BCE_EPS);
-        bsum += -(y * logf(pc + BCE_EPS) + (1.f - y) * logf(1.f - pc + BCE_EPS));
-        if (dsed_pre && live) {
-            const bool pass = (pv >= BCE_EPS) && (pv <= 1.f - BCE_EPS);
-            const float dldp = pass ? -(y / (pc + BCE_EPS) - (1.f - y) / (1.f - pc + BCE_EPS)) : 0.f;
-            dsed_pre[(size_t)r * ld_sed + c] = coef_sed * dldp * pv * (1.f - pv);
-        }
-    }
-    const float* d = doa + (size_t)r * 3 * nc;
-    const float* yd = y_doa + (size_t)r * 3 * nc;
-    float dsum = 0.f;
-    if (doa_loss != 1) {
-        const float inv = 1.f / (float)(3 * nc);
-        for (int k = q; k < 3 * nc; k += 4) {
-            const float pk = d[k], yk = yd[k];
-            float term, dldp;
-            if (doa_loss == 0) {
-                const float e = yk - pk;
-                term = e * e;
-                dldp = -2.f * e;
-            } else if (doa_loss == 2) {
-                const float e = pk - yk;
-                term = fabsf(e);
-                dldp = e > 0.f ? 1.f : (e < 0.f ? -1.f : 0.f);
-            } else {
-                const float lp = logf(fmaxf(pk, BCE_EPS) + 1.f), ly = logf(fmaxf(yk, BCE_EPS) + 1.f);
-                const float e = lp - ly;
-                term = e * e;
-                const float pass = pk > BCE_EPS ? 1.f : (pk == BCE_EPS ? 0.5f : 0.f);
-                dldp = 2.f * e * pass / (fmaxf(pk, BCE_EPS) + 1.f);
-            }
-            dsum += term;
-            if (ddoa_pre && live) ddoa_pre[(size_t)r * ld_doa + k] = w_doa * (dldp * inv) * (1.f - pk * pk);
-        }
-        dsum = loss_quad_sum(dsum) * inv;
-        if (dloss_rows && live && q == 0) dloss_rows[r] = dsum;
-    } else {
-        const float den = den_dev[0];
-        for (int c = q; c < nc; c += 4) {
-            const float a = yd[c], b = yd[nc + c], e3 = yd[2 * nc + c];
-            const float m = rintf(a * a + b * b + e3 * e3);
-            for (int k = 0; k < 3; ++k) {
-                const int i = k * nc + c;
-                const float e = yd[i] - d[i];
-                dsum += e * e * m;
-                if (ddoa_pre && live) ddoa_pre[(size_t)r * ld_doa + i] = w_doa * (-2.f * e * m / den) * (1.f - d[i] * d[i]);
-            }
-        }
-        dsum = loss_quad_sum(dsum);
-    }
-    bsum = loss_quad_sum(bsum);
-    if (q == 0) { rs[rl][0] = live ? bsum : 0.f; rs[rl][1] = live ? dsum : 0.f; }
-    __syncthreads();
-    if (threadIdx.x < 2) {
-        double s = 0.0;
-        for (int i = 0; i < 64; ++i) s += (double)rs[i][threadIdx.x];
-        blockpart[(size_t)blockIdx.x * 2 + threadIdx.x] = s;
-    }
+    float bsum, dsum;
+    loss_row_terms(sed + (size_t)r * nc, doa + (size_t)r * 3 * nc, y_sed + (size_t)r * nc, y_doa + (size_t)r * 3 * nc, doa_loss, coef_sed, w_doa,
+                   den_dev, dloss_rows ? dloss_rows + r : nullptr, dsed_pre ? dsed_pre + (size_t)r * ld_sed : nullptr,
+                   ddoa_pre ? ddoa_pre + (size_t)r * ld_doa : nullptr, nullptr, nullptr, nc, q, live, bsum, dsum);
+    loss_block_sums(rs, bsum, dsum, q, rl, live, blockpart);
 }
 
 __global__ __launch_bounds__(64) void losses_finalize_kernel(const double* __restrict__ blockpart, int nblocks, int doa_loss, double n_sed,
@@ -137,6 +72,9 @@
     if (doa_loss == 1 && dloss) dloss[0] = (float)(s1 / (double)den_dev[0]);
 }
 
+float losses_coef_sed(float w_sed, float sed_grad_scale, int doa_loss, int rows, int nc) {
+    return w_sed * sed_grad_scale * (doa_loss != 1 ? (float)rows : 1.f) / ((float)rows * (float)nc);
+}
 int launch_losses_finalize(hipStream_t st, int doa_loss, const float* den_dev, float* sloss, float* dloss, float* scratch, int B, int S,
                            int nc);
 int launch_losses(hipStream_t st, const float* sed, const float* doa, const float* y_sed, const float* y_doa,
@@ -146,7 +84,7 @@
     if (ld_sed <= 0) ld_sed = nc;
     if (ld_doa <= 0) ld_doa = 3 * nc;
     const int rows = B * S;
-    const float coef_sed = w_sed * sed_grad_scale * (doa_loss != 1 ? (float)rows : 1.f) / ((float)rows * (float)nc);
+    const float coef_sed = losses_coef_sed(w_sed, sed_grad_scale, doa_loss, rows, nc);
     double* blockpart = reinterpret_cast<double*>(scratch);
     const int nblocks = (rows + 63) / 64;
     hipLaunchKernelGGL(losses_kernel, dim3(nblocks), dim3(256), 0, st, sed, doa, y_sed, y_doa, doa_loss, coef_sed, w_doa, den_dev,
diff --git a/seld_amd/csrc/loss_rows.h b/seld_amd/csrc/loss_rows.h
--- /dev/null
+++ b/seld_amd/csrc/loss_rows.h
@@ -0,0 +1,94 @@
+#pragma once
+#include "common.h"
+
+#define BCE_EPS 1e-7f
+
+__device__ __forceinline__ float loss_quad_sum(float v) {
+    v += __int_as_float(__builtin_amdgcn_update_dpp(0, __float_as_int(v), 0xB1 , 0xF, 0xF, true));
+    v += __int_as_float(__builtin_amdgcn_update_dpp(0, __float_as_int(v), 0x4E , 0xF, 0xF, true));
+    return v;
+}
+
+__device__ __forceinline__ float loss_mul_rn(float a, float b) {
+#pragma clang fp contract(off)
+    return a * b;
+}
+
+#define LOSS_T_LD 65
+__device__ __forceinline__ void loss_row_terms(const float* p, const float* d, const float* ys, const float* yd, int doa_loss, float coef_sed,
+                                               float w_doa, const float* den_dev, float* dloss_row, float* dsed_pre, float* ddoa_pre,
+                                               float* dsed_t, float* ddoa_t, int nc, int q, bool live, float& bsum_out, float& dsum_out) {
+    float bsum = 0.f;
+    for (int c = q; c < nc; c += 4) {
+        const float pv = p[c], y = ys[c];
+        const float pc = fminf(fmaxf(pv, BCE_EPS), 1.f - BCE_EPS);
+        bsum += -(y * logf(pc + BCE_EPS) + (1.f - y) * logf(1.f - pc + BCE_EPS));
+        if (dsed_pre && live) {
+            const bool pass = (pv >= BCE_EPS) && (pv <= 1.f - BCE_EPS);
+            const float dldp = pass ? -(y / (pc + BCE_EPS) - (1.f - y) / (1.f - pc + BCE_EPS)) : 0.f;
+            const float g = coef_sed * dldp * pv * (1.f - pv);
+            dsed_pre[c] = g;
+            if (dsed_t) dsed_t[c * LOSS_T_LD] = g;
+        }
+    }
+    float dsum = 0.f;
+    if (doa_loss != 1) {
+        const float inv = 1.f / (float)(3 * nc);
+        for (int k = q; k < 3 * nc; k += 4) {
+            const float pk = d[k], yk = yd[k];
+            float term, dldp;
+            if (doa_loss == 0) {
+                const float e = yk - pk;
+                term = e * e;
+                dldp = -2.f * e;
+            } else if (doa_loss == 2) {
+                const float e = pk - yk;
+                term = fabsf(e);
+                dldp = e > 0.f ? 1.f : (e < 0.f ? -1.f : 0.f);
+            } else {
+                const float lp = logf(fmaxf(pk, BCE_EPS) + 1.f), ly = logf(fmaxf(yk, BCE_EPS) + 1.f);
+                const float e = lp - ly;
+                term = e * e;
+                const float pass = pk > BCE_EPS ? 1.f : (pk == BCE_EPS ? 0.5f : 0.f);
+                dldp = 2.f * e * pass / (fmaxf(pk, BCE_EPS) + 1.f);
+            }
+            dsum += term;
+            if (ddoa_pre && live) {
+                const float g = w_doa * (dldp * inv) * (1.f - loss_mul_rn(pk, pk));
+                ddoa_pre[k] = g;
+                if (ddoa_t) ddoa_t[k * LOSS_T_LD] = g;
+            }
+        }
+        dsum = loss_quad_sum(dsum) * inv;
+        if (dloss_row && live && q == 0) dloss_row[0] = dsum;
+    } else {
+        const float den = den_dev[0];
+        for (int c = q; c < nc; c += 4) {
+            const float a = yd[c], b = yd[nc + c], e3 = yd[2 * nc + c];
+            const float m = rintf(a * a + b * b + e3 * e3);
+            for (int k = 0; k < 3; ++k) {
+                const int i = k * nc + c;
+                const float e = yd[i] - d[i];
+                dsum += e * e * m;
+                if (ddoa_pre && live) {
+                    const float g = w_doa * (-2.f * e * m / den) * (1.f - d[i] * d[i]);
+                    ddoa_pre[i] = g;
+                    if (ddoa_t) ddoa_t[i * LOSS_T_LD] = g;
+                }
+            }
+        }
+        dsum = loss_quad_sum(dsum);
+    }
+    bsum_out = loss_quad_sum(bsum);
+    dsum_out = dsum;
+}
+
+__device__ __forceinline__ void loss_block_sums(float (*rs)[2], float bsum, float dsum, int q, int rl, bool live, double* __restrict__ blockpart) {
+    if (q == 0) { rs[rl][0] = live ? bsum : 0.f; rs[rl][1] = live ? dsum : 0.f; }
+    __syncthreads();
+    if (threadIdx.x < 2) {
+        double s = 0.0;
+        for (int i = 0; i < 64; ++i) s += (double)rs[i][threadIdx.x];
+        blockpart[(size_t)blockIdx.x * 2 + threadIdx.x] = s;
+    }
+}
```
